# 82magnolia/piccolo

Hardware: AMD Instinct MI355X
Metric: candidate-poses/s (higher is better)
Workload: dtype f32

## Files before the change

__graft_entry__.py:

```python
import os
import sys

REPO = os.path.dirname(os.path.abspath(__file__))
if REPO not in sys.path:
    sys.path.insert(0, REPO)


def build():
    import torch
    from piccolo_amd import build as hip_build
    so = hip_build.build()
    assert os.path.exists(so), so
    assert os.path.exists(hip_build.build_experiments())
    from oracle import oracle as orc
    orc.build()
    from piccolo_amd import _lib
    lib = _lib.load()
    assert lib.pcl_abi_version() == _lib.ABI_VERSION
    import piccolo_amd


def smoke():
    import numpy as np
    import torch
    from oracle import oracle as orc
    from piccolo_amd import _lib, ops, synth
    from piccolo_amd import omniloc as po

    assert torch.cuda.is_available(), "smoke() needs the MI355X"
    _lib.load()
    n, H, W, B = 20_000, 128, 256, 4
    xyz, rgb = synth.box_room(n, 1)
    t_gt, ypr_gt = synth.gt_pose(1)
    dev = torch.device("cuda:0")
    X, C = torch.from_numpy(xyz).to(dev), torch.from_numpy(rgb).to(dev)
    cam = ops.transform_cloud(X, torch.from_numpy(t_gt), torch.from_numpy(ypr_gt))
    img = synth.quantise_like_image_file(ops.make_pano(cam, C, (H, W)))
    trans, rot = synth.start_poses(t_gt, ypr_gt, B, seed=1)

    out = ops.sampling_loss(ops.Cloud(X, C), ops.Pano(img), torch.from_numpy(trans), torch.from_numpy(rot)).cpu().numpy()
    img_host = img.cpu().numpy()
    ref = orc.sampling_loss(xyz, rgb, img_host, trans, rot, dtype=np.float64)
    ref32 = orc.sampling_loss(xyz, rgb, img_host, trans, rot, dtype=np.float32)

    def rel(a, b):
        return np.abs(a - b).max() / np.abs(b).max()

    assert rel(out[:, 0], ref["loss"]) <= 5e-7, (out[:, 0], ref["loss"])
    for key, cols in (("grad_t", slice(2, 5)), ("grad_ypr", slice(5, 8))):
        gap = rel(ref32[key], ref[key])
        err = rel(out[:, cols], ref[key])
        assert err <= 2 * gap + 5e-6, (key, err, gap)

    class Cfg:
        lr, num_iter, patience, factor, out_of_room_quantile, num_input = 0.1, 5, 5, 0.8, 0.05, B

    res = po.omniloc_batch(img, X, C, torch.from_numpy(trans).to(dev), torch.from_numpy(rot).to(dev), Cfg(), {})
    assert res[0].shape == (3, 1) and res[1].shape == (3, 3) and torch.isfinite(res[2])
    print("smoke ok: loss", out[:, 0], "-> refined loss", float(res[2]))


if __name__ == "__main__":
    build()
    if "--smoke" in sys.argv:
        smoke()
```

piccolo_amd/build.py:

```python
import glob
import os
import subprocess
import sys

HERE = os.path.dirname(os.path.abspath(__file__))
CSRC = os.path.join(HERE, "csrc")
OUT_DIR = os.path.join(HERE, "lib")
SO = os.path.join(OUT_DIR, "libpiccolo_hip.so")
ARCH = "gfx950"


def hipcc():
    for c in (os.environ.get("HIPCC"), "/opt/rocm/bin/hipcc", "hipcc"):
        if c and (os.path.isabs(c) and os.path.exists(c) or not os.path.isabs(c)):
            return c
    return "hipcc"


def sources():
    return sorted(glob.glob(os.path.join(CSRC, "*.hip")))


def loss_kernel_source_hash():
    import hashlib
    h = hashlib.sha256()
    for name in ("pcl_loss.hip", "pcl_sample_device.h", "pcl_gd_device.h", "pcl_device.h"):
        with open(os.path.join(CSRC, name), "rb") as f:
            h.update(f.read())
    return h.hexdigest()[:16]


def library_source_hash():
    import hashlib
    h = hashlib.sha256()
    for path in sorted(glob.glob(os.path.join(CSRC, "*.hip")) + glob.glob(os.path.join(CSRC, "*.h"))) + [os.path.join(HERE, "..", "include", "piccolo_hip.h")]:
        with open(path, "rb") as f:
            h.update(f.read())
    return h.hexdigest()[:16]


EXP_SO = os.path.join(OUT_DIR, "libpiccolo_hip_exp.so")
HASH_FILE = "pcl_pack.hip"


def _deps():
    return sources() + glob.glob(os.path.join(CSRC, "*.h")) + [os.path.join(HERE, "..", "include", "piccolo_hip.h")]


def stale(so=None):
    so = so or SO
    if not os.path.exists(so):
        return True
    t = os.path.getmtime(so)
    return any(os.path.getmtime(d) > t for d in _deps())


def build(force=False, verbose=False, extra_flags=(), experiments=False):
    from concurrent.futures import ThreadPoolExecutor
    extra_flags = list(extra_flags) + os.environ.get("PCL_HIPCC_FLAGS", "").split()
    so = EXP_SO if experiments else SO
    if not force and not stale(so):
        return so
    obj_dir = os.path.join(OUT_DIR, "obj_exp" if experiments else "obj")
    os.makedirs(obj_dir, exist_ok=True)
    base = [hipcc(), "--offload-arch=" + ARCH, "-O3", "-std=c++17", "-fPIC", "-fno-gpu-rdc", "-pthread", "-Wall", "-Wno-unused-function"]
    base += (["-DPCL_EXPERIMENTS"] if experiments else []) + extra_flags
    hashes = ['-DPCL_SOURCE_HASH="%s"' % loss_kernel_source_hash(), '-DPCL_LIBRARY_HASH="%s"' % library_source_hash()]
    newest_header = max(os.path.getmtime(d) for d in _deps() if not d.endswith(".hip"))

    def compile_one(src):
        obj = os.path.join(obj_dir, os.path.basename(src)[:-4] + ".o")
        stamped = os.path.basename(src) == HASH_FILE
        if not force and not stamped and not extra_flags and os.path.exists(obj) and os.path.getmtime(obj) > max(os.path.getmtime(src), newest_header):
            return obj
        cmd = base + (hashes if stamped else []) + ["-c", src, "-o", obj]
        if verbose:
            print(" ".join(cmd), flush=True)
        subprocess.check_call(cmd)
        return obj

    with ThreadPoolExecutor(max_workers=min(8, os.cpu_count() or 1)) as pool:
        objs = list(pool.map(compile_one, sources()))
    cmd = [hipcc(), "--offload-arch=" + ARCH, "-shared", "-fPIC", "-fno-gpu-rdc", "-pthread", "-o", so] + objs
    if verbose:
        print(" ".join(cmd), flush=True)
    subprocess.check_call(cmd)
    return so


def build_experiments(force=False, verbose=False):
    return build(force=force, verbose=verbose, experiments=True)


if __name__ == "__main__":
    print(build(force="--force" in sys.argv, verbose=True, experiments="--experiments" in sys.argv))
```

piccolo_amd/csrc/pcl_device.h:

```cpp
#pragma once
#include <hip/hip_runtime.h>
#include <stddef.h>
#include <stdint.h>

#include "../../include/piccolo_hip.h"

#ifdef PCL_EXPERIMENTS
#include <stdlib.h>
static inline int pcl_knob_read(const char* name, int dflt)
{
    const char* v = getenv(name);
    return v && *v ? atoi(v) : dflt;
}
#define PCL_KNOB(NAME, dflt) pcl_knob_read("PCL_" #NAME, (dflt))
#else
#define PCL_KNOB(NAME, dflt) (dflt)
#endif

#define PCL_WAVE 64
#define PCL_BLOCK 256
#define PCL_NACC 8

typedef float pcl_f4 __attribute__((ext_vector_type(4)));
typedef int pcl_i4 __attribute__((ext_vector_type(4)));
typedef int pcl_i2 __attribute__((ext_vector_type(2)));

struct PclPoseRec {
    float R[9];
    float t[3];
    uint32_t pano_lo, pano_hi;
    uint32_t cset;
    float pad;
};
static_assert(sizeof(PclPoseRec) == 64, "pose record is one 64-byte scalar-load line");
static_assert(offsetof(PclPoseRec, R) == 0 && offsetof(PclPoseRec, t) == 36, "pose record: t directly after R[9]");

struct PclGdPose {
    double lr;
    double best;
    float leaf[6];
    float fwd[6];
    float m[6];
    float v[6];
    float last_loss;
    int32_t num_bad;
    int32_t step;
    int32_t pad;
    double beta1_pow, beta2_pow;
    float sc[4];
};
static_assert(sizeof(PclGdPose) == 160, "GD state record");

struct PclDims {
    int H, W;
    int Wp;
    float half_w, half_h;
    float off_x, off_y;
    float k_phi, k_theta;
    float c_scale;
    float k_ix, k_iy;
};

__host__ __device__ inline PclDims pcl_make_dims(int H, int W, int pano_format = PCL_PANO_F32)
{
    PclDims d;
    d.H = H; d.W = W; d.Wp = W + 2;
    d.half_w = 0.5f * (float)W; d.half_h = 0.5f * (float)H;
    d.off_x = 0.5f * (float)(W - 1) + 1.0f; d.off_y = 0.5f * (float)(H - 1) + 1.0f;
    d.k_phi = (float)(-(double)W / (2.0 * 3.14159265358979323846));
    d.k_theta = (float)((double)H / 3.14159265358979323846);
    d.c_scale = 1.0f;
    d.k_ix = (float)(-(double)W / (2.0 * 3.14159265358979323846));
    d.k_iy = (float)(-(double)H / 3.14159265358979323846);
    if (pano_format == PCL_PANO_U8 || pano_format == PCL_PANO_F16) {
        d.k_phi = (float)(-(double)W / (2.0 * 3.14159265358979323846) / 255.0);
        d.k_theta = (float)((double)H / 3.14159265358979323846 / 255.0);
        d.c_scale = (float)(1.0 / 255.0);
    }
    return d;
}

struct PclDepthGrid {
    int Hd, Wd, last;
    float wm1, hm1;
    float tol2;
};
__host__ __device__ inline PclDepthGrid pcl_make_depth_grid(int Hd, int Wd, float tau)
{
    PclDepthGrid g;
    g.Hd = Hd; g.Wd = Wd; g.last = Hd * Wd - 1;
    g.wm1 = (float)(Wd - 1); g.hm1 = (float)(Hd - 1);
    g.tol2 = (1.0f + tau) * (1.0f + tau);
    return g;
}
struct PclDepthLook {
    const uint32_t* zbuf;
    PclDepthGrid grid;
    uint32_t* zclear;
    int64_t zclear_vec4;
};
__device__ inline void pcl_rot_from_ypr(float yaw, float pitch, float roll, float R[9])
{
    double sy, cy, sp, cp, sr, cr;
    sincos((double)yaw, &sy, &cy);
    sincos((double)pitch, &sp, &cp);
    sincos((double)roll, &sr, &cr);
    sy = (double)(float)sy; cy = (double)(float)cy; sp = (double)(float)sp;
    cp = (double)(float)cp; sr = (double)(float)sr; cr = (double)(float)cr;
    R[0] = (float)(cy * cp); R[1] = (float)(cy * sp * sr - sy * cr); R[2] = (float)(cy * sp * cr + sy * sr);
    R[3] = (float)(sy * cp); R[4] = (float)(sy * sp * sr + cy * cr); R[5] = (float)(sy * sp * cr - cy * sr);
    R[6] = (float)(-sp);     R[7] = (float)(cp * sr);                R[8] = (float)(cp * cr);
}

__device__ inline void pcl_write_pose_rec(PclPoseRec* rec, const float p[6])
{
    float R[9];
    pcl_rot_from_ypr(p[3], p[4], p[5], R);
    for (int k = 0; k < 9; k++) rec->R[k] = R[k];
    rec->t[0] = p[0]; rec->t[1] = p[1]; rec->t[2] = p[2];
    rec->pano_lo = 0u; rec->pano_hi = 0u;
    rec->cset = 0u; rec->pad = 0.f;
}

__device__ inline void pcl_write_pose_rec_fast(PclPoseRec* rec, const float p[6], float sc[4])
{
    float sy, cy, sp, cp, sr, cr;
    sincosf(p[3], &sy, &cy);
    sincosf(p[4], &sp, &cp);
    sincosf(p[5], &sr, &cr);
    double dsy = sy, dcy = cy, dsp = sp, dcp = cp, dsr = sr, dcr = cr;
    rec->R[0] = (float)(dcy * dcp); rec->R[1] = (float)(dcy * dsp * dsr - dsy * dcr); rec->R[2] = (float)(dcy * dsp * dcr + dsy * dsr);
    rec->R[3] = (float)(dsy * dcp); rec->R[4] = (float)(dsy * dsp * dsr + dcy * dcr); rec->R[5] = (float)(dsy * dsp * dcr - dcy * dsr);
    rec->R[6] = (float)(-dsp);      rec->R[7] = (float)(dcp * dsr);                   rec->R[8] = (float)(dcp * dcr);
    rec->t[0] = p[0]; rec->t[1] = p[1]; rec->t[2] = p[2];
    sc[0] = sy; sc[1] = cy; sc[2] = sp; sc[3] = cp;
}

__device__ inline void pcl_cloud2idx_point(float px, float py, float pz, float& gx, float& gy)
{
#pragma clang fp contract(off)
    const float pi = 3.14159265358979323846f, two_pi = 6.28318530717958647692f;
    float rho = sqrtf(px * px + py * py);
    float theta = atan2f(rho, pz + 1e-6f);
    float phi = atan2f(py, px + 1e-6f) + pi;
    float cx = 1.0f - phi / two_pi;
    float cy = theta / pi;
    gx = 2.0f * cx - 1.0f;
    gy = 2.0f * cy - 1.0f;
}

__device__ __forceinline__ float pcl_atan_poly(float t)
{
    float s = t * t;
    float p = 2.4566929979e-03f;
    p = fmaf(p, s, -1.4401224869e-02f);
    p = fmaf(p, s, 3.9780993102e-02f);
    p = fmaf(p, s, -7.2348362183e-02f);
    p = fmaf(p, s, 1.0498935044e-01f);
    p = fmaf(p, s, -1.4161225936e-01f);
    p = fmaf(p, s, 1.9985906258e-01f);
    p = fmaf(p, s, -3.3332596993e-01f);
    p = fmaf(p, s, 9.9999988638e-01f);
    return p * t;
}

__device__ __forceinline__ float pcl_atan2(float y, float x)
{
    const float pi = 3.14159265358979323846f, half_pi = 1.57079632679489661923f;
    float ax = fabsf(x), ay = fabsf(y);
    float mx = fmaxf(fmaxf(ax, ay), 1e-37f), mn = fminf(ax, ay);
    float r = pcl_atan_poly(mn * __builtin_amdgcn_rcpf(mx));
    r = ay > ax ? half_pi - r : r;
    r = x < 0.f ? pi - r : r;
    return copysignf(r, y);
}

__device__ __forceinline__ float pcl_atan2_ypos(float y, float x)
{
    const float pi = 3.14159265358979323846f, half_pi = 1.57079632679489661923f;
    float ax = fabsf(x);
    float mx = fmaxf(fmaxf(ax, y), 1e-37f), mn = fminf(ax, y);
    float r = pcl_atan_poly(mn * __builtin_amdgcn_rcpf(mx));
    r = y > ax ? half_pi - r : r;
    return x < 0.f ? pi - r : r;
}

__device__ inline __amdgpu_buffer_rsrc_t pcl_tex_rsrc(const void* pano, int H, int W, int texel_bytes = 16)
{
    return __builtin_amdgcn_make_buffer_rsrc((void*)pano, 0, (int)((size_t)(H + 2) * (size_t)(W + 2) * (size_t)texel_bytes),
                                             0x00020000);
}

__host__ __device__ constexpr int pcl_texel_bytes(int fmt) { return fmt == PCL_PANO_U8 ? 4 : fmt == PCL_PANO_F16 ? 8 : 16; }

__device__ inline pcl_i2 pcl_texel_pair_u8(__amdgpu_buffer_rsrc_t rsrc, int voff, int soff)
{
    return __builtin_amdgcn_raw_buffer_load_b64(rsrc, voff, soff, 0);
}
__device__ __forceinline__ float pcl_ub0(int v) { float f; asm("v_cvt_f32_ubyte0 %0, %1" : "=v"(f) : "v"(v)); return f; }
__device__ __forceinline__ float pcl_ub1(int v) { float f; asm("v_cvt_f32_ubyte1 %0, %1" : "=v"(f) : "v"(v)); return f; }
__device__ __forceinline__ float pcl_ub2(int v) { float f; asm("v_cvt_f32_ubyte2 %0, %1" : "=v"(f) : "v"(v)); return f; }

__device__ inline pcl_f4 pcl_texel(__amdgpu_buffer_rsrc_t rsrc, int voff, int soff)
{
    pcl_i4 v = __builtin_amdgcn_raw_buffer_load_b128(rsrc, voff, soff, 0);
    return __builtin_bit_cast(pcl_f4, v);
}

template <int CTRL>
__device__ __forceinline__ float pcl_dpp(float v)
{
    return __builtin_bit_cast(float, __builtin_amdgcn_update_dpp(0, __builtin_bit_cast(int, v), CTRL, 0xf, 0xf, true));
}
__device__ __forceinline__ float pcl_wave_sum(float v)
{
    v += pcl_dpp<0xB1>(v);
    v += pcl_dpp<0x4E>(v);
    v += pcl_dpp<0x141>(v);
    v += pcl_dpp<0x140>(v);
    float r0 = __builtin_bit_cast(float, __builtin_amdgcn_readlane(__builtin_bit_cast(int, v), 0));
    float r1 = __builtin_bit_cast(float, __builtin_amdgcn_readlane(__builtin_bit_cast(int, v), 16));
    float r2 = __builtin_bit_cast(float, __builtin_amdgcn_readlane(__builtin_bit_cast(int, v), 32));
    float r3 = __builtin_bit_cast(float, __builtin_amdgcn_readlane(__builtin_bit_cast(int, v), 48));
    return (r0 + r1) + (r2 + r3);
}

template <int CTRL>
__device__ __forceinline__ double pcl_dpp_d(double v)
{
    pcl_i2 w = __builtin_bit_cast(pcl_i2, v);
    w.x = __builtin_amdgcn_update_dpp(0, w.x, CTRL, 0xf, 0xf, true);
    w.y = __builtin_amdgcn_update_dpp(0, w.y, CTRL, 0xf, 0xf, true);
    return __builtin_bit_cast(double, w);
}
__device__ __forceinline__ double pcl_readlane_d(double v, int lane)
{
    pcl_i2 w = __builtin_bit_cast(pcl_i2, v);
    w.x = __builtin_amdgcn_readlane(w.x, lane);
    w.y = __builtin_amdgcn_readlane(w.y, lane);
    return __builtin_bit_cast(double, w);
}
__device__ __forceinline__ double pcl_wave_sum_d(double v)
{
    v += pcl_dpp_d<0xB1>(v);
    v += pcl_dpp_d<0x4E>(v);
    v += pcl_dpp_d<0x141>(v);
    v += pcl_dpp_d<0x140>(v);
    return (pcl_readlane_d(v, 0) + pcl_readlane_d(v, 16)) + (pcl_readlane_d(v, 32) + pcl_readlane_d(v, 48));
}

#define PCL_LAUNCH_CHECK()                         \
    do {                                           \
        hipError_t e_ = hipGetLastError();         \
        if (e_ != hipSuccess) return (int)e_;      \
    } while (0)
```

piccolo_amd/csrc/pcl_loss.hip:

```cpp
#include <stdlib.h>

#include "pcl_gd_device.h"
#include "pcl_sample_device.h"

struct PclLossArgs {
    const float* cloud;
    int64_t n, stride;
    const void* pano;
    PclDims dims;
    const PclPoseRec* poses;
    int B;
    const uint8_t* visible;
    const uint32_t* zbuf;
    PclDepthGrid dgrid;
    pcl_i4* zclear;
    int zclear_per_block;
    int64_t zclear_total;
    float* partials;
    int nchunks;
    int ngroups;
    int flip;
    int seg_len;
    int xcd_groups;
    int steps_base, steps_rem;
    int color_sets;
};

#define PCL_STEP (2 * PCL_BLOCK)

#ifdef PCL_BLOCK_TRACE
__device__ unsigned long long* pcl_trace_buf = nullptr;
extern "C" int pcl_debug_set_block_trace(unsigned long long* buf)
{
    return (int)hipMemcpyToSymbol(HIP_SYMBOL(pcl_trace_buf), &buf, sizeof(buf));
}
#define PCL_TRACE_NOW() __builtin_amdgcn_s_memrealtime()
__global__ void pcl_debug_stamp_kernel(unsigned long long* slot) { *slot = PCL_TRACE_NOW(); }
extern "C" int pcl_debug_stamp(unsigned long long* slot, void* stream)
{
    hipLaunchKernelGGL(pcl_debug_stamp_kernel, dim3(1), dim3(1), 0, (hipStream_t)stream, slot);
    return (int)hipGetLastError();
}
#endif

template <int G, bool FUSED>
__device__ __forceinline__ unsigned pcl_room_select(const PclLossArgs& a_in, const PclFuseArgs& f_in, const PclRoomTable* __restrict__ tb, PclLossArgs& a,
                                                    PclFuseArgs& f)
{
    int r = -1;
#pragma unroll
    for (int q = 0; q < PCL_GD_MAX_ROOMS; q++) r += (int)blockIdx.x >= pcl_rfl(tb->block0[q]) ? 1 : 0;
    const PclRoomRec* __restrict__ rm = tb->rec + r;
    const int group0 = pcl_rfl(rm->group0), pose0 = group0 * G;
    const long long poff = (long long)pcl_rfl64((unsigned long long)rm->partials);
    a = a_in;
    a.cloud = (const float*)pcl_rfl64(rm->cloud);
    a.n = pcl_rfl(rm->n); a.stride = pcl_rfl(rm->stride);
    a.nchunks = pcl_rfl(rm->nchunks); a.seg_len = pcl_rfl(rm->seg_len);
    a.steps_base = pcl_rfl(rm->steps_base); a.steps_rem = pcl_rfl(rm->steps_rem);
    a.poses = a_in.poses + pose0;
    a.partials = a_in.partials + poff;
    a.xcd_groups = 0;
    f = f_in;
    if constexpr (FUSED) {
        f.partials_in = f_in.partials_in + poff;
        f.st_in = f_in.st_in + pose0; f.recs_in = f_in.recs_in + pose0;
        f.st_out = f_in.st_out + pose0; f.recs_out = f_in.recs_out + pose0;
        f.box = (const float*)pcl_rfl64(rm->box);
        f.loss_out = f_in.loss_out ? f_in.loss_out + pose0 : nullptr;
    }
    return blockIdx.x - (unsigned)pcl_rfl(rm->block0);
}

template <int G, bool GRAD, int VIS, int FMT, bool FUSED, bool CS = false, bool RM = false>
__device__ __forceinline__ void pcl_loss_body(const PclLossArgs& a_in, const PclFuseArgs& f_in, const PclRoomTable* rooms = nullptr)
{
    PclLossArgs a_rm;
    PclFuseArgs f_rm;
    unsigned bid = blockIdx.x;
    if constexpr (RM) bid = pcl_room_select<G, FUSED>(a_in, f_in, rooms, a_rm, f_rm);
    const PclLossArgs& a = RM ? a_rm : a_in;
    const PclFuseArgs& f = RM ? f_rm : f_in;
    int group, chunk;
    if (a.xcd_groups) {
        const int gpx = a.ngroups >> 3, j = (int)(bid >> 3), cj = j / gpx;
        group = (int)(bid & 7) * gpx + (j - cj * gpx);
        chunk = a.flip ? a.nchunks - 1 - cj : cj;
    } else {
        const int lq = (int)(bid >> 3) / a.ngroups;
        group = (int)(bid >> 3) - lq * a.ngroups;
        const int lc = a.flip ? (a.nchunks >> 3) - 1 - lq : lq;
        const int run = lc / a.seg_len;
        chunk = (run * 8 + (int)(bid & 7)) * a.seg_len + (lc - run * a.seg_len);
    }
    const int pose0 = group * G;

    PclPose6 P6[G];
    unsigned PANO[G][2];
    __amdgpu_buffer_rsrc_t tex = pcl_tex_rsrc(a.pano, a.dims.H, a.dims.W, pcl_texel_bytes(FMT));
    __amdgpu_buffer_rsrc_t cld = __builtin_amdgcn_make_buffer_rsrc((void*)a.cloud, 0, CS ? (int)(a.stride * (3 + 3 * a.color_sets) * 4) : (int)(a.stride * 6 * 4),
                                                                   0x00020000);
    const int plane = (int)a.stride * 4;
    int cplane = 3 * plane;
    if constexpr (CS) cplane = (int)(3u + 3u * (unsigned)__builtin_amdgcn_readfirstlane((int)(a.poses + pose0)->cset)) * plane;
    __amdgpu_buffer_rsrc_t zb = __amdgpu_buffer_rsrc_t();
    if constexpr (VIS == 2) zb = __builtin_amdgcn_make_buffer_rsrc((void*)a.zbuf, 0, (int)((unsigned)a.B * (unsigned)(a.dgrid.last + 1) * 4u), 0x00020000);

    f2 acc[G][PCL_NACC];
    int count[G];
#pragma unroll
    for (int g = 0; g < G; g++) {
        count[g] = 0;
#pragma unroll
        for (int k = 0; k < PCL_NACC; k++) acc[g][k] = F2(0.f);
    }

    int first = chunk * a.steps_base + min(chunk, a.steps_rem);
    int nsteps = a.steps_base + (chunk < a.steps_rem ? 1 : 0);
    const int begin = first * PCL_STEP;
    int end = begin + nsteps * PCL_STEP;
    if (end > (int)a.n) end = (int)a.n;
    const int last = (int)a.n - 1;

    auto load_step = [&](int base, float (&dst)[2][6]) {
        int j0 = min(base + (int)threadIdx.x, last), j1 = min(base + PCL_BLOCK + (int)threadIdx.x, last);
#pragma unroll
        for (int k = 0; k < 6; k++) {
            const int soff = (CS && k >= 3) ? cplane + (k - 3) * plane : k * plane;
            dst[0][k] = __builtin_bit_cast(float, __builtin_amdgcn_raw_buffer_load_b32(cld, j0 * 4, soff, 0));
            dst[1][k] = __builtin_bit_cast(float, __builtin_amdgcn_raw_buffer_load_b32(cld, j1 * 4, soff, 0));
        }
    };
    auto eval_step = [&](int base, const float (&src)[2][6]) {
        const int i0 = base + threadIdx.x, i1 = i0 + PCL_BLOCK;
        const bool valid0 = i0 < end, valid1 = i1 < end;
        const unsigned long long vmask0 = __builtin_amdgcn_ballot_w64(valid0), vmask1 = __builtin_amdgcn_ballot_w64(valid1);
        f2 x = {src[0][0], src[1][0]}, y = {src[0][1], src[1][1]}, z = {src[0][2], src[1][2]};
        f2 ncr = {src[0][3], src[1][3]}, ncg = {src[0][4], src[1][4]}, ncb = {src[0][5], src[1][5]};
#ifndef PCL_NO_ROTATE_PAIR
        f2 rot_p[G][3];
#ifdef PCL_TIMING_ONLY_NO_ROTATION
        if constexpr (G == 2) {
            const f2 oa = F2((a.poses + pose0)->t[0]), ob = F2((a.poses + pose0 + 1)->t[0]);
            rot_p[0][0] = x - oa; rot_p[0][1] = y; rot_p[0][2] = z;
            rot_p[1][0] = x - ob; rot_p[1][1] = y; rot_p[1][2] = z;
        } else
#endif
        if constexpr (G == 2) {
            if constexpr (FUSED) pcl_rotate2x2(x, y, z, P6[0], P6[1], rot_p[0][0], rot_p[0][1], rot_p[0][2], rot_p[1][0], rot_p[1][1], rot_p[1][2]);
            else pcl_rotate2x2(x, y, z, pcl_pose6(a.poses + pose0), pcl_pose6(a.poses + pose0 + 1), rot_p[0][0], rot_p[0][1], rot_p[0][2],
                               rot_p[1][0], rot_p[1][1], rot_p[1][2]);
        }
#endif
#pragma unroll
        for (int g = 0; g < G; g++) {
            const PclPoseRec* __restrict__ pr = a.poses + (pose0 + g);
            bool ok0 = valid0, ok1 = valid1;
            unsigned long long m0 = vmask0, m1 = vmask1;
            if constexpr (VIS == 1) {
                const uint8_t* vis = a.visible + (int64_t)(pose0 + g) * a.n;
                ok0 = ok0 && vis[min(i0, last)] != 0;
                ok1 = ok1 && vis[min(i1, last)] != 0;
                m0 = __builtin_amdgcn_ballot_w64(ok0); m1 = __builtin_amdgcn_ballot_w64(ok1);
            }
            __amdgpu_buffer_rsrc_t tg = tex;
            unsigned pano_lo = pr->pano_lo, pano_hi = pr->pano_hi;
            if constexpr (FUSED) {
                pano_lo = PANO[g][0]; pano_hi = PANO[g][1];
            }
            if (pano_lo | pano_hi) {
                const void* pp = (const void*)(((unsigned long long)pano_hi << 32) | (unsigned long long)pano_lo);
                tg = pcl_tex_rsrc(pp, a.dims.H, a.dims.W, pcl_texel_bytes(FMT));
            }
            PclProj<FMT> pj;
            const int zoff = VIS == 2 ? (int)((unsigned)(pose0 + g) * (unsigned)(a.dgrid.last + 1) * 4u) : 0;
#ifndef PCL_NO_ROTATE_PAIR
            if constexpr (G == 2) {
                pj.px = rot_p[g][0]; pj.py = rot_p[g][1]; pj.pz = rot_p[g][2];
                pcl_project2_rotated<FMT, VIS == 2>(tg, a.dims, pj, zb, zoff, &a.dgrid);
            } else
#endif
            if constexpr (FUSED) pcl_project2<FMT, VIS == 2>(x, y, z, P6[g], tg, a.dims, pj, zb, zoff, &a.dgrid);
            else pcl_project2<FMT, VIS == 2>(x, y, z, pcl_pose6(pr), tg, a.dims, pj, zb, zoff, &a.dgrid);
            if constexpr (VIS == 2) {
                f2 d2 = pcl_fma2(pj.pz, pj.pz, pj.rho2);
                const bool v0 = d2.x <= __uint_as_float(pj.zq0), v1 = d2.y <= __uint_as_float(pj.zq1);
                ok0 = ok0 & v0; ok1 = ok1 & v1;
                m0 = __builtin_amdgcn_ballot_w64(ok0); m1 = __builtin_amdgcn_ballot_w64(ok1);
            }
            pcl_sample2<GRAD, FMT>(pj, ncr, ncg, ncb, ok0, ok1, m0, m1, tg, a.dims, acc[g], count[g]);
        }
    };
    float bufA[2][6], bufB[2][6];
    load_step(begin, bufA);
    if constexpr (FUSED) {
        static_assert(PCL_BLOCK == PCL_GD_THREADS, "the fused prologue reduces with the epilogue kernel's thread layout");
        __shared__ double gd_rows[(PCL_GD_THREADS / 16) * 2 * G][4];
        __shared__ double gd_sums[G][PCL_NACC];
        __shared__ float pose_sh[G][12];
        pcl_gd_finish_group<G, true>(f.partials_in, a.nchunks, group, (int)threadIdx.x, f.st_in, f.recs_in, f.st_out, f.recs_out, chunk == 0,
                                     f.box, f.factor, f.patience, f.mode, f.loss_out, gd_rows, gd_sums, pose_sh);
        __syncthreads();
#pragma unroll
        for (int g = 0; g < G; g++) {
            float v[12];
#pragma unroll
            for (int k = 0; k < 12; k++) v[k] = __builtin_bit_cast(float, __builtin_amdgcn_readfirstlane(__builtin_bit_cast(int, pose_sh[g][k])));
            P6[g] = PclPose6{(f2){v[0], v[1]}, (f2){v[2], v[3]}, (f2){v[4], v[5]}, (f2){v[6], v[7]}, (f2){v[8], v[9]}, (f2){v[10], v[11]}};
            const PclPoseRec* pr = a.poses + (pose0 + g);
            PANO[g][0] = (unsigned)__builtin_amdgcn_readfirstlane((int)pr->pano_lo);
            PANO[g][1] = (unsigned)__builtin_amdgcn_readfirstlane((int)pr->pano_hi);
        }
    }

    for (int base = begin; base < end; base += 2 * PCL_STEP) {
        load_step(base + PCL_STEP, bufB);
        eval_step(base, bufA);
        if (base + PCL_STEP < end) {
            load_step(base + 2 * PCL_STEP, bufA);
            eval_step(base + PCL_STEP, bufB);
        }
    }

    __shared__ float red[PCL_BLOCK / PCL_WAVE][G * PCL_NACC];
    const int lane = threadIdx.x & 63, wave = threadIdx.x >> 6;
#pragma unroll
    for (int g = 0; g < G; g++)
#pragma unroll
        for (int k = 0; k < PCL_NACC; k++) {
            if (k == 1) {
                if (lane == 0) red[wave][g * PCL_NACC + 1] = (float)count[g];
                continue;
            }
            if (!GRAD && k >= 2) continue;
            float s = pcl_wave_sum(acc[g][k].x + acc[g][k].y);
            if (lane == 0) red[wave][g * PCL_NACC + k] = s;
        }
    __syncthreads();
    if (threadIdx.x < G * PCL_NACC) {
        int g = threadIdx.x / PCL_NACC, k = threadIdx.x - g * PCL_NACC;
        float s = 0.f;
        if (GRAD || k < 2) s = red[0][threadIdx.x] + red[1][threadIdx.x] + red[2][threadIdx.x] + red[3][threadIdx.x];
        a.partials[pcl_partials_row(a.nchunks, G, group, chunk, g) + k] = s;
    }
    if constexpr (VIS == 2) {
        if (a.zclear) {
            const pcl_i4 inf4 = {0x7f800000, 0x7f800000, 0x7f800000, 0x7f800000};
            const int64_t z0 = (int64_t)blockIdx.x * a.zclear_per_block;
            for (int i = threadIdx.x; i < a.zclear_per_block; i += PCL_BLOCK)
                if (z0 + i < a.zclear_total) a.zclear[z0 + i] = inf4;
        }
    }
#ifdef PCL_BLOCK_TRACE
    if (pcl_trace_buf && threadIdx.x == 0) {
        unsigned hw, xcc;
        asm volatile("s_getreg_b32 %0, hwreg(HW_REG_HW_ID)" : "=s"(hw));
        asm volatile("s_getreg_b32 %0, hwreg(HW_REG_XCC_ID)" : "=s"(xcc));
        unsigned long long* t = pcl_trace_buf + (size_t)blockIdx.x * 4;
        t[0] = 0; t[1] = 0; t[2] = PCL_TRACE_NOW(); t[3] = ((unsigned long long)xcc << 32) | hw;
    }
#endif
}

template <int G, bool GRAD, int VIS, int FMT>
__global__ void __launch_bounds__(PCL_BLOCK) pcl_loss_kernel(PclLossArgs a)
{
    pcl_loss_body<G, GRAD, VIS, FMT, false>(a, PclFuseArgs{});
}

template <int G, int FMT>
__global__ void __launch_bounds__(PCL_BLOCK) pcl_loss_fused_kernel(PclLossArgs a, PclFuseArgs f)
{
    pcl_loss_body<G, true, 0, FMT, true>(a, f);
}

template <int G, int FMT>
__global__ void __launch_bounds__(PCL_BLOCK) pcl_loss_sets_kernel(PclLossArgs a)
{
    pcl_loss_body<G, true, 0, FMT, false, true>(a, PclFuseArgs{});
}

template <int G, int FMT>
__global__ void __launch_bounds__(PCL_BLOCK) pcl_loss_fused_sets_kernel(PclLossArgs a, PclFuseArgs f)
{
    pcl_loss_body<G, true, 0, FMT, true, true>(a, f);
}

template <int G, int FMT>
__global__ void __launch_bounds__(PCL_BLOCK) pcl_loss_rooms_kernel(PclLossArgs a, const PclRoomTable* rooms)
{
    pcl_loss_body<G, true, 0, FMT, false, false, true>(a, PclFuseArgs{}, rooms);
}

template <int G, int FMT>
__global__ void __launch_bounds__(PCL_BLOCK) pcl_loss_fused_rooms_kernel(PclLossArgs a, PclFuseArgs f, const PclRoomTable* rooms)
{
    pcl_loss_body<G, true, 0, FMT, true, false, true>(a, f, rooms);
}



struct PclPlan {
    int G, ngroups, nchunks;
    int seg_len;
    int steps_base, steps_rem;
};

static int pcl_xcd_seg_len(int nchunks, int64_t nblocks)
{
    static const int runs_env = PCL_KNOB(XCD_RUNS, 0);
    int cpx = nchunks / 8, runs = runs_env < 1 || runs_env > cpx ? cpx : runs_env;
    if (runs_env < 1 && nblocks <= 1024) runs = 1;
    while (cpx % runs) runs--;
    return cpx / runs;
}

static PclPlan pcl_plan(int64_t n, int B)
{
    static const int g_env = PCL_KNOB(G, 0), blocks_env = PCL_KNOB(BLOCKS, 4096);
    PclPlan p;
    p.G = (B % 2 == 0) ? 2 : 1;
    if (g_env > 0 && B % g_env == 0) p.G = g_env;
    p.ngroups = B / p.G;
    int64_t want = blocks_env / p.ngroups;
    if (want < 64) want = 64;
    if (n > 2000000 && want < n / 8192) want = n / 8192;
    int64_t steps = (n + PCL_STEP - 1) / PCL_STEP;
    if (steps < 3 * want) {
        int64_t alt = steps / 3;
        if (alt < 1024 / p.ngroups) alt = 1024 / p.ngroups;
        if (alt < 32) alt = 32;
        if (alt < want) want = alt;
    }
    if (want > steps) want = steps;
    want = ((want + 7) / 8) * 8;
    p.nchunks = (int)want;
    p.steps_base = (int)(steps / want);
    p.steps_rem = (int)(steps % want);
    p.seg_len = pcl_xcd_seg_len(p.nchunks, (int64_t)p.nchunks * p.ngroups);
    return p;
}

static PclPlan pcl_plan_sets(int64_t n, int B, int sets)
{
    if (sets <= 1) return pcl_plan(n, B);
    PclPlan p = pcl_plan(n, B / sets);
    p.ngroups = B / p.G;
    p.seg_len = pcl_xcd_seg_len(p.nchunks, (int64_t)p.nchunks * p.ngroups);
    return p;
}

void pcl_plan_room(int64_t n, int per_room, int* G, int* ngroups, int* nchunks, int* seg_len, int* steps_base, int* steps_rem)
{
    const PclPlan p = pcl_plan(n, per_room);
    *G = p.G; *ngroups = p.ngroups; *nchunks = p.nchunks; *seg_len = p.seg_len; *steps_base = p.steps_base; *steps_rem = p.steps_rem;
}

size_t pcl_partials_bytes(int64_t n, int B, int sets)
{
    PclPlan p = pcl_plan_sets(n, B, sets);
    return (size_t)p.nchunks * (size_t)B * PCL_NACC * sizeof(float);
}

int pcl_plan_nchunks(int64_t n, int B, int sets) { return pcl_plan_sets(n, B, sets).nchunks; }
int pcl_plan_nblocks(int64_t n, int B, int sets) { PclPlan p = pcl_plan_sets(n, B, sets); return p.nchunks * p.ngroups; }
int pcl_plan_G(int64_t n, int B, int sets) { return pcl_plan_sets(n, B, sets).G; }

void pcl_plan_for_groups(int64_t n, int ngroups, int* nchunks, int* seg_len, int* steps_base, int* steps_rem)
{
    PclPlan p = pcl_plan(n, 2 * ngroups);
    static const int chunks_env = PCL_KNOB(TRIM_CHUNKS, 0);
    int auto_chunks = 0;
    const int64_t per_chunk = n <= 2000000 ? 8192 : 16384;
    if (chunks_env < 8 && n > 64 * per_chunk) auto_chunks = (int)((n + per_chunk - 1) / per_chunk);
    if (chunks_env >= 8 || auto_chunks) {
        int64_t steps = (n + PCL_STEP - 1) / PCL_STEP, want = (((chunks_env >= 8 ? chunks_env : auto_chunks) + 7) / 8) * 8;
        if (want > steps) want = ((steps + 7) / 8) * 8;
        p.nchunks = (int)want; p.steps_base = (int)(steps / want); p.steps_rem = (int)(steps % want);
        static const int runs_env = PCL_KNOB(TRIM_RUNS, 0);
        int cpx = p.nchunks / 8, runs = runs_env < 1 || runs_env > cpx ? cpx : runs_env;
        while (cpx % runs) runs--;
        p.seg_len = cpx / runs;
    }
    *nchunks = p.nchunks; *seg_len = p.seg_len; *steps_base = p.steps_base; *steps_rem = p.steps_rem;
}

template <int G, int FMT>
static void pcl_launch_g(const PclLossArgs& a, int nblk, bool grad, int vis, hipStream_t s)
{
    if (grad) {
        if (vis == 2) hipLaunchKernelGGL((pcl_loss_kernel<G, true, 2, FMT>), dim3(nblk), dim3(PCL_BLOCK), 0, s, a);
        else if (vis) hipLaunchKernelGGL((pcl_loss_kernel<G, true, 1, FMT>), dim3(nblk), dim3(PCL_BLOCK), 0, s, a);
        else hipLaunchKernelGGL((pcl_loss_kernel<G, true, 0, FMT>), dim3(nblk), dim3(PCL_BLOCK), 0, s, a);
    } else {
        if (vis == 2) hipLaunchKernelGGL((pcl_loss_kernel<G, false, 2, FMT>), dim3(nblk), dim3(PCL_BLOCK), 0, s, a);
        else if (vis) hipLaunchKernelGGL((pcl_loss_kernel<G, false, 1, FMT>), dim3(nblk), dim3(PCL_BLOCK), 0, s, a);
        else hipLaunchKernelGGL((pcl_loss_kernel<G, false, 0, FMT>), dim3(nblk), dim3(PCL_BLOCK), 0, s, a);
    }
}

template <int FMT>
static void pcl_launch_f(const PclLossArgs& a, int G, int nblk, bool grad, int vis, hipStream_t s)
{
    if (G == 4) pcl_launch_g<4, FMT>(a, nblk, grad, vis, s);
    else if (G == 2) pcl_launch_g<2, FMT>(a, nblk, grad, vis, s);
    else pcl_launch_g<1, FMT>(a, nblk, grad, vis, s);
}

template <int FMT>
static void pcl_launch_fused(const PclLossArgs& a, const PclFuseArgs& f, int G, int nblk, hipStream_t s)
{
    if (G == 4) hipLaunchKernelGGL((pcl_loss_fused_kernel<4, FMT>), dim3(nblk), dim3(PCL_BLOCK), 0, s, a, f);
    else if (G == 2) hipLaunchKernelGGL((pcl_loss_fused_kernel<2, FMT>), dim3(nblk), dim3(PCL_BLOCK), 0, s, a, f);
    else hipLaunchKernelGGL((pcl_loss_fused_kernel<1, FMT>), dim3(nblk), dim3(PCL_BLOCK), 0, s, a, f);
}

template <int FMT>
static void pcl_launch_sets(const PclLossArgs& a, const PclFuseArgs* f, int G, int nblk, hipStream_t s)
{
    if (f) {
        if (G == 4) hipLaunchKernelGGL((pcl_loss_fused_sets_kernel<4, FMT>), dim3(nblk), dim3(PCL_BLOCK), 0, s, a, *f);
        else if (G == 2) hipLaunchKernelGGL((pcl_loss_fused_sets_kernel<2, FMT>), dim3(nblk), dim3(PCL_BLOCK), 0, s, a, *f);
        else hipLaunchKernelGGL((pcl_loss_fused_sets_kernel<1, FMT>), dim3(nblk), dim3(PCL_BLOCK), 0, s, a, *f);
    } else {
        if (G == 4) hipLaunchKernelGGL((pcl_loss_sets_kernel<4, FMT>), dim3(nblk), dim3(PCL_BLOCK), 0, s, a);
        else if (G == 2) hipLaunchKernelGGL((pcl_loss_sets_kernel<2, FMT>), dim3(nblk), dim3(PCL_BLOCK), 0, s, a);
        else hipLaunchKernelGGL((pcl_loss_sets_kernel<1, FMT>), dim3(nblk), dim3(PCL_BLOCK), 0, s, a);
    }
}

int pcl_launch_loss_rooms(const PclRoomTable* rooms, const void* pano, int pano_format, int H, int W, const PclPoseRec* poses, int B, int G,
                          int ngroups, int nblk, float* partials, hipStream_t s, int flip, const PclFuseArgs* fuse)
{
    if (pano_format != PCL_PANO_F32 && pano_format != PCL_PANO_U8 && pano_format != PCL_PANO_F16) return PCL_EINVAL;
    if ((int64_t)(H + 2) * (W + 2) * pcl_texel_bytes(pano_format) >= ((int64_t)1 << 31)) return PCL_EINVAL;
    PclLossArgs a = PclLossArgs{};
    a.pano = pano; a.dims = pcl_make_dims(H, W, pano_format);
    a.poses = poses; a.B = B; a.partials = partials;
    a.ngroups = ngroups; a.flip = flip & 1; a.xcd_groups = 0; a.color_sets = 1;
    const dim3 grid(nblk), blk(PCL_BLOCK);
    if (fuse) {
        if (pano_format == PCL_PANO_U8) {
            if (G == 2) hipLaunchKernelGGL((pcl_loss_fused_rooms_kernel<2, PCL_PANO_U8>), grid, blk, 0, s, a, *fuse, rooms);
            else hipLaunchKernelGGL((pcl_loss_fused_rooms_kernel<1, PCL_PANO_U8>), grid, blk, 0, s, a, *fuse, rooms);
        } else if (pano_format == PCL_PANO_F16) {
            if (G == 2) hipLaunchKernelGGL((pcl_loss_fused_rooms_kernel<2, PCL_PANO_F16>), grid, blk, 0, s, a, *fuse, rooms);
            else hipLaunchKernelGGL((pcl_loss_fused_rooms_kernel<1, PCL_PANO_F16>), grid, blk, 0, s, a, *fuse, rooms);
        } else {
            if (G == 2) hipLaunchKernelGGL((pcl_loss_fused_rooms_kernel<2, PCL_PANO_F32>), grid, blk, 0, s, a, *fuse, rooms);
            else hipLaunchKernelGGL((pcl_loss_fused_rooms_kernel<1, PCL_PANO_F32>), grid, blk, 0, s, a, *fuse, rooms);
        }
    } else {
        if (pano_format == PCL_PANO_U8) {
            if (G == 2) hipLaunchKernelGGL((pcl_loss_rooms_kernel<2, PCL_PANO_U8>), grid, blk, 0, s, a, rooms);
            else hipLaunchKernelGGL((pcl_loss_rooms_kernel<1, PCL_PANO_U8>), grid, blk, 0, s, a, rooms);
        } else if (pano_format == PCL_PANO_F16) {
            if (G == 2) hipLaunchKernelGGL((pcl_loss_rooms_kernel<2, PCL_PANO_F16>), grid, blk, 0, s, a, rooms);
            else hipLaunchKernelGGL((pcl_loss_rooms_kernel<1, PCL_PANO_F16>), grid, blk, 0, s, a, rooms);
        } else {
            if (G == 2) hipLaunchKernelGGL((pcl_loss_rooms_kernel<2, PCL_PANO_F32>), grid, blk, 0, s, a, rooms);
            else hipLaunchKernelGGL((pcl_loss_rooms_kernel<1, PCL_PANO_F32>), grid, blk, 0, s, a, rooms);
        }
    }
    PCL_LAUNCH_CHECK();
    return 0;
}

int pcl_launch_loss(const float* cloud, int64_t n, const void* pano, int pano_format, int H, int W, const PclPoseRec* poses,
                    int B, bool grad, const uint8_t* visible, float* partials, hipStream_t s, int flip, const PclFuseArgs* fuse,
                    const PclDepthLook* depth, int color_sets)
{
    if (pano_format != PCL_PANO_F32 && pano_format != PCL_PANO_U8 && pano_format != PCL_PANO_F16) return PCL_EINVAL;
    if (n > PCL_MAX_POINTS || (int64_t)(H + 2) * (W + 2) * pcl_texel_bytes(pano_format) >= ((int64_t)1 << 31)) return PCL_EINVAL;
    const bool sets = color_sets > 1;
    if (sets && (B % color_sets || !grad || visible || depth || pcl_cloud_sets_bytes(n, color_sets) == 0)) return PCL_EINVAL;
    PclPlan p = pcl_plan_sets(n, B, color_sets);
    PclLossArgs a;
    a.cloud = cloud; a.n = n; a.stride = pcl_cloud_stride(n);
    a.pano = pano; a.dims = pcl_make_dims(H, W, pano_format);
    a.poses = poses; a.B = B; a.visible = visible; a.partials = partials;
    a.zbuf = nullptr; a.dgrid = PclDepthGrid{};
    a.zclear = nullptr; a.zclear_per_block = 0; a.zclear_total = 0;
    if (depth) {
        if (visible || !depth->zbuf || depth->grid.Hd <= 0 || depth->grid.Wd <= 0) return PCL_EINVAL;
        if ((int64_t)B * depth->grid.Hd * depth->grid.Wd * 4 >= ((int64_t)1 << 32)) return PCL_EINVAL;
        a.zbuf = depth->zbuf; a.dgrid = depth->grid;
        if (depth->zclear) {
            const int64_t nblk64 = (int64_t)p.nchunks * p.ngroups;
            a.zclear = (pcl_i4*)depth->zclear;
            a.zclear_total = depth->zclear_vec4;
            a.zclear_per_block = (int)((depth->zclear_vec4 + nblk64 - 1) / nblk64);
        }
    }
    a.nchunks = p.nchunks; a.ngroups = p.ngroups; a.seg_len = p.seg_len; a.flip = flip & 1; a.steps_base = p.steps_base; a.steps_rem = p.steps_rem;
    a.color_sets = sets ? color_sets : 1;
    static const int xg_env = PCL_KNOB(XCD_GROUPS, -1);
    a.xcd_groups = ((flip & 2) != 0 || xg_env == 1) && xg_env != 0 && p.ngroups % 8 == 0 ? 1 : 0;
    int nblk = p.nchunks * p.ngroups;
    const int vis = depth ? 2 : visible != nullptr ? 1 : 0;
    if (sets) {
        if (pano_format == PCL_PANO_U8) pcl_launch_sets<PCL_PANO_U8>(a, fuse, p.G, nblk, s);
        else if (pano_format == PCL_PANO_F16) pcl_launch_sets<PCL_PANO_F16>(a, fuse, p.G, nblk, s);
        else pcl_launch_sets<PCL_PANO_F32>(a, fuse, p.G, nblk, s);
        PCL_LAUNCH_CHECK();
        return 0;
    }
    if (fuse) {
        if (!grad || vis) return PCL_EINVAL;
        if (pano_format == PCL_PANO_U8) pcl_launch_fused<PCL_PANO_U8>(a, *fuse, p.G, nblk, s);
        else if (pano_format == PCL_PANO_F16) pcl_launch_fused<PCL_PANO_F16>(a, *fuse, p.G, nblk, s);
        else pcl_launch_fused<PCL_PANO_F32>(a, *fuse, p.G, nblk, s);
        PCL_LAUNCH_CHECK();
        return 0;
    }
    if (pano_format == PCL_PANO_U8) pcl_launch_f<PCL_PANO_U8>(a, p.G, nblk, grad, vis, s);
    else if (pano_format == PCL_PANO_F16) pcl_launch_f<PCL_PANO_F16>(a, p.G, nblk, grad, vis, s);
    else pcl_launch_f<PCL_PANO_F32>(a, p.G, nblk, grad, vis, s);
    PCL_LAUNCH_CHECK();
    return 0;
}
```

piccolo_amd/csrc/pcl_pack.hip:

```cpp
#include "pcl_device.h"

#include <rocprim/device/device_radix_sort.hpp>

extern "C" int pcl_abi_version(void) { return PCL_ABI_VERSION; }

#ifndef PCL_SOURCE_HASH
#define PCL_SOURCE_HASH "unstamped"
#endif
extern "C" const char* pcl_source_hash(void) { return PCL_SOURCE_HASH; }
#ifndef PCL_LIBRARY_HASH
#define PCL_LIBRARY_HASH "unstamped"
#endif
extern "C" const char* pcl_library_hash(void) { return PCL_LIBRARY_HASH; }

extern "C" const char* pcl_error_string(int code)
{
    if (code == 0) return "success";
    if (code == PCL_EINVAL) return "piccolo_hip: invalid argument";
    if (code == PCL_EWORKSPACE) return "piccolo_hip: workspace too small";
    if (code > 0) return hipGetErrorString((hipError_t)code);
    return "piccolo_hip: unknown error";
}

extern "C" int64_t pcl_cloud_stride(int64_t n) { return n <= 0 ? 0 : ((n + 255) / 256) * 256; }
extern "C" size_t pcl_cloud_bytes(int64_t n) { return (size_t)pcl_cloud_stride(n) * 6 * sizeof(float); }
extern "C" size_t pcl_pano_bytes(int H, int W, int pano_format)
{
    if (H <= 0 || W <= 0) return 0;
    if (pano_format == PCL_PANO_U8P) return (size_t)((H + 3) >> 1) * (size_t)(W + 2) * 8;
    if (pano_format == PCL_PANO_U8V) return (size_t)(H + 2) * (size_t)(W + 2) * 8;
    if (pano_format != PCL_PANO_F32 && pano_format != PCL_PANO_U8 && pano_format != PCL_PANO_F16) return 0;
    return (size_t)(H + 2) * (size_t)(W + 2) * (size_t)pcl_texel_bytes(pano_format);
}

__global__ void __launch_bounds__(PCL_BLOCK) pcl_cloud_pack_kernel(const float* __restrict__ xyz, const float* __restrict__ rgb,
                                                                   const int64_t* __restrict__ order, int64_t n,
                                                                   int64_t stride, float* __restrict__ cloud)
{
    int64_t i = (int64_t)blockIdx.x * PCL_BLOCK + threadIdx.x;
    if (i >= stride) return;
    float v[6] = {0.f, 0.f, 0.f, 0.f, 0.f, 0.f};
    if (i < n) {
        int64_t j = order ? order[i] : i;
        v[0] = xyz[3 * j]; v[1] = xyz[3 * j + 1]; v[2] = xyz[3 * j + 2];
        v[3] = -rgb[3 * j]; v[4] = -rgb[3 * j + 1]; v[5] = -rgb[3 * j + 2];
    }
#pragma unroll
    for (int k = 0; k < 6; k++) cloud[k * stride + i] = v[k];
}

extern "C" int pcl_cloud_pack(const float* xyz, const float* rgb, const int64_t* order, int64_t n, float* cloud, void* stream)
{
    if (!xyz || !rgb || !cloud || n <= 0) return PCL_EINVAL;
    int64_t stride = pcl_cloud_stride(n);
    hipLaunchKernelGGL(pcl_cloud_pack_kernel, dim3((unsigned)(stride / PCL_BLOCK)), dim3(PCL_BLOCK), 0, (hipStream_t)stream,
                       xyz, rgb, order, n, stride, cloud);
    PCL_LAUNCH_CHECK();
    return 0;
}

extern "C" size_t pcl_cloud_sets_bytes(int64_t n, int nsets)
{
    if (n <= 0 || n > PCL_MAX_POINTS || nsets <= 0) return 0;
    if (nsets == 1) return pcl_cloud_bytes(n);
    const int64_t bytes = (int64_t)pcl_cloud_stride(n) * 4 * (3 + 3 * (int64_t)nsets);
    return bytes < ((int64_t)1 << 31) ? (size_t)bytes : 0;
}

#define PCL_PACK_SETS 16
struct PclRgbList { const float* p[PCL_PACK_SETS]; };

__global__ void __launch_bounds__(PCL_BLOCK) pcl_cloud_pack_sets_kernel(const float* __restrict__ xyz, PclRgbList rgb, int k0, int m,
                                                                        const int64_t* __restrict__ order, int64_t n, int64_t stride,
                                                                        float* __restrict__ cloud)
{
    int64_t i = (int64_t)blockIdx.x * PCL_BLOCK + threadIdx.x;
    if (i >= stride) return;
    const int64_t j = i < n ? (order ? order[i] : i) : 0;
    if (k0 == 0)
        for (int c = 0; c < 3; c++) cloud[c * stride + i] = i < n ? xyz[3 * j + c] : 0.f;
    for (int k = 0; k < m; k++)
        for (int c = 0; c < 3; c++) cloud[(3 + 3 * (int64_t)(k0 + k) + c) * stride + i] = i < n ? -rgb.p[k][3 * j + c] : 0.f;
}

extern "C" int pcl_cloud_pack_sets(const float* xyz, const float* const* rgb_host, int nsets, const int64_t* order, int64_t n, float* cloud,
                                   void* stream)
{
    if (!xyz || !rgb_host || !cloud || n <= 0 || nsets <= 0) return PCL_EINVAL;
    if (pcl_cloud_sets_bytes(n, nsets) == 0) return PCL_EINVAL;
    for (int k = 0; k < nsets; k++)
        if (!rgb_host[k]) return PCL_EINVAL;
    if (nsets == 1) return pcl_cloud_pack(xyz, rgb_host[0], order, n, cloud, stream);
    const int64_t stride = pcl_cloud_stride(n);
    for (int k0 = 0; k0 < nsets; k0 += PCL_PACK_SETS) {
        const int m = nsets - k0 < PCL_PACK_SETS ? nsets - k0 : PCL_PACK_SETS;
        PclRgbList l;
        for (int k = 0; k < PCL_PACK_SETS; k++) l.p[k] = k < m ? rgb_host[k0 + k] : nullptr;
        hipLaunchKernelGGL(pcl_cloud_pack_sets_kernel, dim3((unsigned)(stride / PCL_BLOCK)), dim3(PCL_BLOCK), 0, (hipStream_t)stream, xyz, l, k0, m,
                           order, n, stride, cloud);
        PCL_LAUNCH_CHECK();
    }
    return 0;
}

__device__ inline uint64_t pcl_spread21(uint32_t v)
{
    uint64_t x = v & 0x1fffffu;
    x = (x | x << 32) & 0x1f00000000ffffull;
    x = (x | x << 16) & 0x1f0000ff0000ffull;
    x = (x | x << 8) & 0x100f00f00f00f00full;
    x = (x | x << 4) & 0x10c30c30c30c30c3ull;
    x = (x | x << 2) & 0x1249249249249249ull;
    return x;
}

__global__ void __launch_bounds__(PCL_BLOCK) pcl_morton_kernel(const float* __restrict__ xyz, int64_t n, float lx, float ly,
                                                               float lz, float sx, float sy, float sz,
                                                               int64_t* __restrict__ keys)
{
    int64_t i = (int64_t)blockIdx.x * PCL_BLOCK + threadIdx.x;
    if (i >= n) return;
    const float top = 2097151.f;
    float fx = __builtin_amdgcn_fmed3f((xyz[3 * i] - lx) * sx, 0.f, top);
    float fy = __builtin_amdgcn_fmed3f((xyz[3 * i + 1] - ly) * sy, 0.f, top);
    float fz = __builtin_amdgcn_fmed3f((xyz[3 * i + 2] - lz) * sz, 0.f, top);
    uint64_t k = pcl_spread21((uint32_t)fx) | (pcl_spread21((uint32_t)fy) << 1) | (pcl_spread21((uint32_t)fz) << 2);
    keys[i] = (int64_t)k;
}

extern "C" int pcl_morton_keys(const float* xyz, int64_t n, const float* lo, const float* hi, int64_t* keys, void* stream)
{
    if (!xyz || !lo || !hi || !keys || n <= 0) return PCL_EINVAL;
    float s[3];
    for (int k = 0; k < 3; k++) s[k] = hi[k] > lo[k] ? 2097151.f / (hi[k] - lo[k]) : 0.f;
    hipLaunchKernelGGL(pcl_morton_kernel, dim3((unsigned)((n + PCL_BLOCK - 1) / PCL_BLOCK)), dim3(PCL_BLOCK), 0,
                       (hipStream_t)stream, xyz, n, lo[0], lo[1], lo[2], s[0], s[1], s[2], keys);
    PCL_LAUNCH_CHECK();
    return 0;
}

__device__ __forceinline__ unsigned int pcl_ordered_key(float v)
{
    unsigned int b = __float_as_uint(v);
    return (b & 0x80000000u) ? ~b : (b | 0x80000000u);
}
__device__ __forceinline__ float pcl_ordered_value(unsigned int k)
{
    return __uint_as_float((k & 0x80000000u) ? (k & 0x7fffffffu) : ~k);
}

__global__ void __launch_bounds__(PCL_BLOCK) pcl_bbox_kernel(const float* __restrict__ xyz, int64_t n, unsigned int* __restrict__ box)
{
    unsigned int lo[3] = {~0u, ~0u, ~0u}, hi[3] = {0u, 0u, 0u};
    for (int64_t i = (int64_t)blockIdx.x * PCL_BLOCK + threadIdx.x; i < n; i += (int64_t)gridDim.x * PCL_BLOCK) {
#pragma unroll
        for (int c = 0; c < 3; c++) {
            unsigned int k = pcl_ordered_key(xyz[3 * i + c]);
            lo[c] = min(lo[c], k); hi[c] = max(hi[c], k);
        }
    }
#pragma unroll
    for (int c = 0; c < 3; c++) {
#pragma unroll
        for (int o = 32; o > 0; o >>= 1) {
            lo[c] = min(lo[c], (unsigned int)__shfl_xor((int)lo[c], o, 64));
            hi[c] = max(hi[c], (unsigned int)__shfl_xor((int)hi[c], o, 64));
        }
        if ((threadIdx.x & 63) == 0) { atomicMin(&box[c], lo[c]); atomicMax(&box[3 + c], hi[c]); }
    }
}

__global__ void __launch_bounds__(PCL_BLOCK) pcl_morton_box_kernel(const float* __restrict__ xyz, int64_t n, const unsigned int* __restrict__ box,
                                                                   unsigned long long* __restrict__ keys, int64_t* __restrict__ iota)
{
    int64_t i = (int64_t)blockIdx.x * PCL_BLOCK + threadIdx.x;
    if (i >= n) return;
    const float top = 2097151.f;
    unsigned long long k = 0ull;
#pragma unroll
    for (int c = 0; c < 3; c++) {
        float lo = pcl_ordered_value(box[c]), hi = pcl_ordered_value(box[3 + c]);
        float sc = hi > lo ? top / (hi - lo) : 0.f;
        float f = __builtin_amdgcn_fmed3f((xyz[3 * i + c] - lo) * sc, 0.f, top);
        k |= pcl_spread21((uint32_t)f) << c;
    }
    keys[i] = k;
    iota[i] = i;
}

static size_t order_align(size_t v) { return (v + 255) & ~(size_t)255; }
static size_t order_sort_temp_bytes(int64_t n)
{
    size_t bytes = 0;
    (void)rocprim::radix_sort_pairs<rocprim::default_config, const unsigned long long*, unsigned long long*, const int64_t*, int64_t*>(
        nullptr, bytes, nullptr, nullptr, nullptr, nullptr, (size_t)n, 0, 63, nullptr, false);
    return bytes;
}

extern "C" size_t pcl_cloud_order_workspace_bytes(int64_t n)
{
    if (n <= 0) return 0;
    return order_align(64) + 3 * order_align((size_t)n * 8) + order_align(order_sort_temp_bytes(n));
}

extern "C" int pcl_cloud_order(const float* xyz, int64_t n, int64_t* order, void* workspace, size_t workspace_bytes, void* stream)
{
    if (!xyz || !order || !workspace || n <= 0 || n > PCL_MAX_POINTS) return PCL_EINVAL;
    if (workspace_bytes < pcl_cloud_order_workspace_bytes(n)) return PCL_EWORKSPACE;
    hipStream_t s = (hipStream_t)stream;
    char* ws = (char*)workspace;
    unsigned int* box = (unsigned int*)ws; ws += order_align(64);
    unsigned long long* keys = (unsigned long long*)ws; ws += order_align((size_t)n * 8);
    unsigned long long* keys_sorted = (unsigned long long*)ws; ws += order_align((size_t)n * 8);
    int64_t* iota = (int64_t*)ws; ws += order_align((size_t)n * 8);
    hipError_t e = hipMemsetAsync(box, 0xff, 12, s);
    if (e == hipSuccess) e = hipMemsetAsync(box + 3, 0, 12, s);
    if (e != hipSuccess) return (int)e;
    int64_t blocks = (n + PCL_BLOCK - 1) / PCL_BLOCK;
    hipLaunchKernelGGL(pcl_bbox_kernel, dim3((unsigned)(blocks < 1024 ? blocks : 1024)), dim3(PCL_BLOCK), 0, s, xyz, n, box);
    hipLaunchKernelGGL(pcl_morton_box_kernel, dim3((unsigned)blocks), dim3(PCL_BLOCK), 0, s, xyz, n, box, keys, iota);
    PCL_LAUNCH_CHECK();
    size_t temp_bytes = order_sort_temp_bytes(n);
    e = rocprim::radix_sort_pairs(ws, temp_bytes, (const unsigned long long*)keys, keys_sorted, (const int64_t*)iota, order, (size_t)n, 0, 63,
                                  s, false);
    return e == hipSuccess ? 0 : (int)e;
}

__global__ void __launch_bounds__(PCL_BLOCK) pcl_pano_pack_kernel(const float* __restrict__ img, int H, int W,
                                                                  pcl_f4* __restrict__ pano)
{
    int Wp = W + 2, Hp = H + 2;
    int64_t i = (int64_t)blockIdx.x * PCL_BLOCK + threadIdx.x;
    if (i >= (int64_t)Wp * Hp) return;
    int yp = (int)(i / Wp), xp = (int)(i - (int64_t)yp * Wp);
    pcl_f4 v = {0.f, 0.f, 0.f, 0.f};
    if (yp >= 1 && yp <= H && xp >= 1 && xp <= W) {
        const float* s = img + ((int64_t)(yp - 1) * W + (xp - 1)) * 3;
        v.x = s[0]; v.y = s[1]; v.z = s[2];
    }
    pano[i] = v;
}

extern "C" int pcl_pano_pack(const float* img_hwc, int H, int W, float* pano, void* stream)
{
    if (!img_hwc || !pano || H <= 0 || W <= 0) return PCL_EINVAL;
    int64_t total = (int64_t)(H + 2) * (W + 2);
    hipLaunchKernelGGL(pcl_pano_pack_kernel, dim3((unsigned)((total + PCL_BLOCK - 1) / PCL_BLOCK)), dim3(PCL_BLOCK), 0,
                       (hipStream_t)stream, img_hwc, H, W, (pcl_f4*)pano);
    PCL_LAUNCH_CHECK();
    return 0;
}

__global__ void __launch_bounds__(PCL_BLOCK) pcl_pano_pack_u8_kernel(const float* __restrict__ img, int H, int W,
                                                                     uint32_t* __restrict__ pano, int* __restrict__ not_exact)
{
    int Wp = W + 2, Hp = H + 2;
    int64_t i = (int64_t)blockIdx.x * PCL_BLOCK + threadIdx.x;
    if (i >= (int64_t)Wp * Hp) return;
    int yp = (int)(i / Wp), xp = (int)(i - (int64_t)yp * Wp);
    uint32_t v = 0u;
    if (yp >= 1 && yp <= H && xp >= 1 && xp <= W) {
        const float* s = img + ((int64_t)(yp - 1) * W + (xp - 1)) * 3;
        bool bad = false;
#pragma unroll
        for (int c = 0; c < 3; c++) {
            float f = s[c], k = rintf(f * 255.f);
            bad = bad || !(k >= 0.f && k <= 255.f) || __fdiv_rn(k, 255.f) != f;
            v |= ((uint32_t)k & 255u) << (8 * c);
        }
        if (bad) *not_exact = 1;
    }
    pano[i] = v;
}

__global__ void __launch_bounds__(PCL_BLOCK) pcl_pano_pack_u8p_kernel(const float* __restrict__ img, int H, int W,
                                                                      uint32_t* __restrict__ pano, int* __restrict__ not_exact)
{
    const int Wp = W + 2, pairs = (H + 3) >> 1;
    int64_t i = (int64_t)blockIdx.x * PCL_BLOCK + threadIdx.x;
    if (i >= (int64_t)Wp * pairs * 2) return;
    const int yp = (int)(i / Wp), xp = (int)(i - (int64_t)yp * Wp);
    uint32_t v = 0u;
    if (yp >= 1 && yp <= H && xp >= 1 && xp <= W) {
        const float* s = img + ((int64_t)(yp - 1) * W + (xp - 1)) * 3;
        bool bad = false;
#pragma unroll
        for (int c = 0; c < 3; c++) {
            float f = s[c], k = rintf(f * 255.f);
            bad = bad || !(k >= 0.f && k <= 255.f) || __fdiv_rn(k, 255.f) != f;
            v |= ((uint32_t)k & 255u) << (8 * c);
        }
        if (bad) *not_exact = 1;
    }
    pano[((int64_t)(yp >> 1) * Wp + xp) * 2 + (yp & 1)] = v;
}

__global__ void __launch_bounds__(PCL_BLOCK) pcl_pano_pack_u8v_kernel(const float* __restrict__ img, int H, int W,
                                                                      pcl_i2* __restrict__ pano, int* __restrict__ not_exact)
{
    const int Wp = W + 2, Hp = H + 2;
    int64_t i = (int64_t)blockIdx.x * PCL_BLOCK + threadIdx.x;
    if (i >= (int64_t)Wp * Hp) return;
    const int yp = (int)(i / Wp), xp = (int)(i - (int64_t)yp * Wp);
    uint32_t v[2] = {0u, 0u};
    bool bad = false;
#pragma unroll
    for (int d = 0; d < 2; d++) {
        const int y = yp + d;
        if (y >= 1 && y <= H && xp >= 1 && xp <= W) {
            const float* s = img + ((int64_t)(y - 1) * W + (xp - 1)) * 3;
#pragma unroll
            for (int c = 0; c < 3; c++) {
                float f = s[c], k = rintf(f * 255.f);
                bad = bad || !(k >= 0.f && k <= 255.f) || __fdiv_rn(k, 255.f) != f;
                v[d] |= ((uint32_t)k & 255u) << (8 * c);
            }
        }
    }
    if (bad) *not_exact = 1;
    pano[i] = (pcl_i2){(int)v[0], (int)v[1]};
}

extern "C" int pcl_pano_pack_u8v(const float* img_hwc, int H, int W, uint32_t* pano, int* not_exact, void* stream)
{
    if (!img_hwc || !pano || !not_exact || H <= 0 || W <= 0) return PCL_EINVAL;
    int64_t total = (int64_t)(H + 2) * (W + 2);
    hipLaunchKernelGGL(pcl_pano_pack_u8v_kernel, dim3((unsigned)((total + PCL_BLOCK - 1) / PCL_BLOCK)), dim3(PCL_BLOCK), 0,
                       (hipStream_t)stream, img_hwc, H, W, (pcl_i2*)pano, not_exact);
    PCL_LAUNCH_CHECK();
    return 0;
}

__global__ void __launch_bounds__(PCL_BLOCK) pcl_pano_pack_f16_kernel(const float* __restrict__ img, int H, int W,
                                                                      pcl_i2* __restrict__ pano, int* __restrict__ not_exact)
{
    typedef _Float16 h2 __attribute__((ext_vector_type(2)));
    int Wp = W + 2, Hp = H + 2;
    int64_t i = (int64_t)blockIdx.x * PCL_BLOCK + threadIdx.x;
    if (i >= (int64_t)Wp * Hp) return;
    int yp = (int)(i / Wp), xp = (int)(i - (int64_t)yp * Wp);
    float lv[3] = {0.f, 0.f, 0.f};
    if (yp >= 1 && yp <= H && xp >= 1 && xp <= W) {
        const float* s = img + ((int64_t)(yp - 1) * W + (xp - 1)) * 3;
        bool bad = false;
#pragma unroll
        for (int c = 0; c < 3; c++) {
            float f = s[c], k = rintf(f * 255.f);
            bad = bad || !(k >= 0.f && k <= 255.f) || __fdiv_rn(k, 255.f) != f;
            lv[c] = k;
        }
        if (bad) *not_exact = 1;
    }
    h2 rg = {(_Float16)lv[0], (_Float16)lv[1]}, b0 = {(_Float16)lv[2], (_Float16)0.f};
    pano[i] = (pcl_i2){__builtin_bit_cast(int, rg), __builtin_bit_cast(int, b0)};
}

extern "C" int pcl_pano_pack_f16(const float* img_hwc, int H, int W, void* pano, int* not_exact, void* stream)
{
    if (!img_hwc || !pano || !not_exact || H <= 0 || W <= 0) return PCL_EINVAL;
    int64_t total = (int64_t)(H + 2) * (W + 2);
    hipLaunchKernelGGL(pcl_pano_pack_f16_kernel, dim3((unsigned)((total + PCL_BLOCK - 1) / PCL_BLOCK)), dim3(PCL_BLOCK), 0,
                       (hipStream_t)stream, img_hwc, H, W, (pcl_i2*)pano, not_exact);
    PCL_LAUNCH_CHECK();
    return 0;
}

extern "C" int pcl_pano_pack_u8p(const float* img_hwc, int H, int W, uint32_t* pano, int* not_exact, void* stream)
{
    if (!img_hwc || !pano || !not_exact || H <= 0 || W <= 0) return PCL_EINVAL;
    int64_t total = (int64_t)((H + 3) >> 1) * 2 * (W + 2);
    hipLaunchKernelGGL(pcl_pano_pack_u8p_kernel, dim3((unsigned)((total + PCL_BLOCK - 1) / PCL_BLOCK)), dim3(PCL_BLOCK), 0,
                       (hipStream_t)stream, img_hwc, H, W, pano, not_exact);
    PCL_LAUNCH_CHECK();
    return 0;
}

extern "C" int pcl_pano_pack_u8(const float* img_hwc, int H, int W, uint32_t* pano, int* not_exact, void* stream)
{
    if (!img_hwc || !pano || !not_exact || H <= 0 || W <= 0) return PCL_EINVAL;
    int64_t total = (int64_t)(H + 2) * (W + 2);
    hipLaunchKernelGGL(pcl_pano_pack_u8_kernel, dim3((unsigned)((total + PCL_BLOCK - 1) / PCL_BLOCK)), dim3(PCL_BLOCK), 0,
                       (hipStream_t)stream, img_hwc, H, W, pano, not_exact);
    PCL_LAUNCH_CHECK();
    return 0;
}
```

piccolo_amd/csrc/pcl_sample_device.h:

```cpp
#pragma once
#include "pcl_device.h"

typedef float f2 __attribute__((ext_vector_type(2)));
#define F2(s) ((f2){(s), (s)})

__device__ __forceinline__ f2 pcl_fma2(f2 a, f2 b, f2 c) { return __builtin_elementwise_fma(a, b, c); }

__device__ __forceinline__ f2 pcl_atan_poly2(f2 t)
{
    f2 s = t * t;
    f2 p = F2(2.4566929979e-03f);
    p = pcl_fma2(p, s, F2(-1.4401224869e-02f));
    p = pcl_fma2(p, s, F2(3.9780993102e-02f));
    p = pcl_fma2(p, s, F2(-7.2348362183e-02f));
    p = pcl_fma2(p, s, F2(1.0498935044e-01f));
    p = pcl_fma2(p, s, F2(-1.4161225936e-01f));
    p = pcl_fma2(p, s, F2(1.9985906258e-01f));
    p = pcl_fma2(p, s, F2(-3.3332596993e-01f));
    p = pcl_fma2(p, s, F2(9.9999988638e-01f));
    return p * t;
}

__device__ __forceinline__ float pcl_min_abs(float a, float b)
{
    float r;
    asm("v_min_f32_e64 %0, |%1|, |%2|" : "=v"(r) : "v"(a), "v"(b));
    return r;
}
__device__ __forceinline__ f2 pcl_atan_ratio2(float u0, float v0, float u1, float v1)
{
    f2 mn = {pcl_min_abs(u0, v0), pcl_min_abs(u1, v1)};
    f2 rc = {__builtin_amdgcn_rcpf(fmaxf(fmaxf(fabsf(u0), fabsf(v0)), 1e-37f)), __builtin_amdgcn_rcpf(fmaxf(fmaxf(fabsf(u1), fabsf(v1)), 1e-37f))};
    return pcl_atan_poly2(mn * rc);
}

__device__ __forceinline__ f2 pcl_atan2_2(f2 y, f2 x)
{
    const float half_pi = 1.57079632679489661923f;
    float ax0 = fabsf(x.x), ax1 = fabsf(x.y), ay0 = fabsf(y.x), ay1 = fabsf(y.y);
    f2 r = pcl_atan_ratio2(x.x, y.x, x.y, y.y);
    f2 alt = F2(half_pi) - r;
    r = (f2){ay0 > ax0 ? alt.x : r.x, ay1 > ax1 ? alt.y : r.y};
    f2 w = F2(half_pi) - r;
    w = (f2){copysignf(w.x, x.x), copysignf(w.y, x.y)};
    r = F2(half_pi) - w;
    return (f2){copysignf(r.x, y.x), copysignf(r.y, y.y)};
}

__device__ __forceinline__ f2 pcl_elevation2(f2 z, f2 rho)
{
    const float half_pi = 1.57079632679489661923f;
    float az0 = fabsf(z.x), az1 = fabsf(z.y);
    f2 r = pcl_atan_ratio2(rho.x, z.x, rho.y, z.y);
    f2 alt = F2(half_pi) - r;
    r = (f2){az0 > rho.x ? alt.x : r.x, az1 > rho.y ? alt.y : r.y};
    return (f2){copysignf(r.x, z.x), copysignf(r.y, z.y)};
}

template <int FMT> struct PclTaps;
template <> struct PclTaps<PCL_PANO_U8> { pcl_i2 top, bot; };
template <> struct PclTaps<PCL_PANO_F32> { int voff, row; };
template <> struct PclTaps<PCL_PANO_F16> { pcl_i4 top, bot; };

__device__ __forceinline__ void pcl_issue_taps(__amdgpu_buffer_rsrc_t tex, int x0, int y0, int Wp, PclTaps<PCL_PANO_U8>& o)
{
    int voff = (int)(__umul24((unsigned)y0, (unsigned)Wp) + (unsigned)x0) * 4;
    o.top = pcl_texel_pair_u8(tex, voff, 0);
    o.bot = pcl_texel_pair_u8(tex, voff, Wp * 4);
}
__device__ __forceinline__ void pcl_issue_taps(__amdgpu_buffer_rsrc_t tex, int x0, int y0, int Wp, PclTaps<PCL_PANO_F16>& o)
{
    int voff = (int)(__umul24((unsigned)y0, (unsigned)Wp) + (unsigned)x0) * 8;
    o.top = __builtin_amdgcn_raw_buffer_load_b128(tex, voff, 0, 0);
    o.bot = __builtin_amdgcn_raw_buffer_load_b128(tex, voff, Wp * 8, 0);
}
__device__ __forceinline__ void pcl_issue_taps(__amdgpu_buffer_rsrc_t tex, int x0, int y0, int Wp, PclTaps<PCL_PANO_F32>& o)
{
    o.voff = (int)(__umul24((unsigned)y0, (unsigned)Wp) + (unsigned)x0) * 16;
    o.row = Wp * 16;
}
__device__ __forceinline__ void pcl_unpack_taps(__amdgpu_buffer_rsrc_t, const PclTaps<PCL_PANO_U8>& r, float t[12])
{
    t[0] = pcl_ub0(r.top.x); t[1] = pcl_ub1(r.top.x); t[2] = pcl_ub2(r.top.x);
    t[3] = pcl_ub0(r.top.y); t[4] = pcl_ub1(r.top.y); t[5] = pcl_ub2(r.top.y);
    t[6] = pcl_ub0(r.bot.x); t[7] = pcl_ub1(r.bot.x); t[8] = pcl_ub2(r.bot.x);
    t[9] = pcl_ub0(r.bot.y); t[10] = pcl_ub1(r.bot.y); t[11] = pcl_ub2(r.bot.y);
}
__device__ __forceinline__ void pcl_unpack_taps(__amdgpu_buffer_rsrc_t tex, const PclTaps<PCL_PANO_F32>& r, float t[12])
{
    pcl_f4 t00 = pcl_texel(tex, r.voff, 0), t01 = pcl_texel(tex, r.voff + 16, 0);
    pcl_f4 t10 = pcl_texel(tex, r.voff, r.row), t11 = pcl_texel(tex, r.voff + 16, r.row);
    t[0] = t00.x; t[1] = t00.y; t[2] = t00.z; t[3] = t01.x; t[4] = t01.y; t[5] = t01.z;
    t[6] = t10.x; t[7] = t10.y; t[8] = t10.z; t[9] = t11.x; t[10] = t11.y; t[11] = t11.z;
}

typedef _Float16 pcl_h2 __attribute__((ext_vector_type(2)));
__device__ __forceinline__ float pcl_mix_lo(float a, pcl_h2 b, pcl_h2 c)
{
    float r;
    asm("v_fma_mix_f32 %0, %1, %2, %3 op_sel:[0,0,0] op_sel_hi:[0,1,1]" : "=v"(r) : "v"(a), "v"(b), "v"(c));
    return r;
}
__device__ __forceinline__ float pcl_mix_hi(float a, pcl_h2 b, pcl_h2 c)
{
    float r;
    asm("v_fma_mix_f32 %0, %1, %2, %3 op_sel:[0,1,1] op_sel_hi:[0,1,1]" : "=v"(r) : "v"(a), "v"(b), "v"(c));
    return r;
}
struct PclBilerp1 { float top[3], bot[3], dh[3]; };
template <bool GRAD>
__device__ __forceinline__ void pcl_bilerp_f16(const PclTaps<PCL_PANO_F16>& r, float fx, float fy, PclBilerp1& o)
{
    typedef _Float16 pcl_h8 __attribute__((ext_vector_type(8)));
    pcl_h8 tv = __builtin_bit_cast(pcl_h8, r.top), bv = __builtin_bit_cast(pcl_h8, r.bot);
    pcl_h2 t00a = __builtin_shufflevector(tv, tv, 0, 1), t00b = __builtin_shufflevector(tv, tv, 2, 3);
    pcl_h2 t01a = __builtin_shufflevector(tv, tv, 4, 5), t01b = __builtin_shufflevector(tv, tv, 6, 7);
    pcl_h2 t10a = __builtin_shufflevector(bv, bv, 0, 1), t10b = __builtin_shufflevector(bv, bv, 2, 3);
    pcl_h2 t11a = __builtin_shufflevector(bv, bv, 4, 5), t11b = __builtin_shufflevector(bv, bv, 6, 7);
    pcl_h2 dta = t01a - t00a, dtb = t01b - t00b, dba = t11a - t10a, dbb = t11b - t10b;
    o.top[0] = pcl_mix_lo(fx, dta, t00a); o.bot[0] = pcl_mix_lo(fx, dba, t10a);
    o.top[1] = pcl_mix_hi(fx, dta, t00a); o.bot[1] = pcl_mix_hi(fx, dba, t10a);
    o.top[2] = pcl_mix_lo(fx, dtb, t00b); o.bot[2] = pcl_mix_lo(fx, dbb, t10b);
    if (GRAD) {
        pcl_h2 dda = dba - dta, ddb = dbb - dtb;
        o.dh[0] = pcl_mix_lo(fy, dda, dta);
        o.dh[1] = pcl_mix_hi(fy, dda, dta);
        o.dh[2] = pcl_mix_lo(fy, ddb, dtb);
    }
}

template <int FMT>
struct PclProj {
    f2 px, py, pz;
    f2 rho2, rinv;
    f2 rs2;
    f2 fx, fy;
    bool in_phi0, in_phi1, in_th0, in_th1;
    PclTaps<FMT> ta, tb;
    unsigned zq0, zq1;
};

__device__ __forceinline__ void pcl_depth_cells2(f2 phi, f2 hel, const PclDepthGrid& g, int& row0, int& col0, int& row1, int& col1)
{
    const float inv_2pi = 0.15915494309189532f;
    f2 colf = pcl_fma2(-phi, F2(inv_2pi), F2(0.5f)) * F2(g.wm1);
    f2 rowf = pcl_fma2(-(hel * F2(4.0f)), F2(inv_2pi), F2(0.5f)) * F2(g.hm1);
    row0 = (int)rowf.x; col0 = (int)colf.x; row1 = (int)rowf.y; col1 = (int)colf.y;
}

struct PclPose6 { f2 p0, p1, p2, p3, p4, p5; };
__device__ __forceinline__ PclPose6 pcl_pose6(const PclPoseRec* __restrict__ pose)
{
    const f2* __restrict__ P = reinterpret_cast<const f2*>(pose->R);
    return PclPose6{P[0], P[1], P[2], P[3], P[4], P[5]};
}
__device__ __forceinline__ void pcl_rotate2(f2 x, f2 y, f2 z, const PclPose6& P, f2& opx, f2& opy, f2& opz)
{
    const f2 p0 = P.p0, p1 = P.p1, p2 = P.p2, p3 = P.p3, p4 = P.p4, p5 = P.p5;
    f2 qx, qy, qz, px, py, pz;
    asm("v_pk_add_f32 %3, %6, %13 op_sel:[0,1] op_sel_hi:[1,1] neg_lo:[0,1] neg_hi:[0,1]\n\t"
        "v_pk_add_f32 %4, %7, %14 op_sel_hi:[1,0] neg_lo:[0,1] neg_hi:[0,1]\n\t"
        "v_pk_add_f32 %5, %8, %14 op_sel:[0,1] op_sel_hi:[1,1] neg_lo:[0,1] neg_hi:[0,1]\n\t"
        "v_pk_mul_f32 %0, %3, %9 op_sel_hi:[1,0]\n\t"
        "v_pk_mul_f32 %1, %3, %10 op_sel:[0,1] op_sel_hi:[1,1]\n\t"
        "v_pk_mul_f32 %2, %3, %12 op_sel_hi:[1,0]\n\t"
        "v_pk_fma_f32 %0, %9, %4, %0 op_sel:[1,0,0] op_sel_hi:[1,1,1]\n\t"
        "v_pk_fma_f32 %1, %11, %4, %1 op_sel_hi:[0,1,1]\n\t"
        "v_pk_fma_f32 %2, %12, %4, %2 op_sel:[1,0,0] op_sel_hi:[1,1,1]\n\t"
        "v_pk_fma_f32 %0, %10, %5, %0 op_sel_hi:[0,1,1]\n\t"
        "v_pk_fma_f32 %1, %11, %5, %1 op_sel:[1,0,0] op_sel_hi:[1,1,1]\n\t"
        "v_pk_fma_f32 %2, %13, %5, %2 op_sel_hi:[0,1,1]\n\t"
        "s_nop 0"
        : "=&v"(px), "=&v"(py), "=&v"(pz), "=&v"(qx), "=&v"(qy), "=&v"(qz)
        : "v"(x), "v"(y), "v"(z), "s"(p0), "s"(p1), "s"(p2), "s"(p3), "s"(p4), "s"(p5));
    opx = px; opy = py; opz = pz;
}
#ifndef PCL_NO_ROTATE_PAIR
__device__ __forceinline__ void pcl_rotate2x2(f2 x, f2 y, f2 z, const PclPose6& A, const PclPose6& B, f2& apx, f2& apy, f2& apz, f2& bpx,
                                              f2& bpy, f2& bpz)
{
    f2 aqx, aqy, aqz, bqx, bqy, bqz, ax, ay, az, bx, by, bz;
    asm("v_pk_add_f32 %6, %12, %19 op_sel:[0,1] op_sel_hi:[1,1] neg_lo:[0,1] neg_hi:[0,1]\n\t"
        "v_pk_add_f32 %9, %12, %25 op_sel:[0,1] op_sel_hi:[1,1] neg_lo:[0,1] neg_hi:[0,1]\n\t"
        "v_pk_add_f32 %7, %13, %20 op_sel_hi:[1,0] neg_lo:[0,1] neg_hi:[0,1]\n\t"
        "v_pk_add_f32 %10, %13, %26 op_sel_hi:[1,0] neg_lo:[0,1] neg_hi:[0,1]\n\t"
        "v_pk_add_f32 %8, %14, %20 op_sel:[0,1] op_sel_hi:[1,1] neg_lo:[0,1] neg_hi:[0,1]\n\t"
        "v_pk_add_f32 %11, %14, %26 op_sel:[0,1] op_sel_hi:[1,1] neg_lo:[0,1] neg_hi:[0,1]\n\t"
        "v_pk_mul_f32 %0, %6, %15 op_sel_hi:[1,0]\n\t"
        "v_pk_mul_f32 %3, %9, %21 op_sel_hi:[1,0]\n\t"
        "v_pk_mul_f32 %1, %6, %16 op_sel:[0,1] op_sel_hi:[1,1]\n\t"
        "v_pk_mul_f32 %4, %9, %22 op_sel:[0,1] op_sel_hi:[1,1]\n\t"
        "v_pk_mul_f32 %2, %6, %18 op_sel_hi:[1,0]\n\t"
        "v_pk_mul_f32 %5, %9, %24 op_sel_hi:[1,0]\n\t"
        "v_pk_fma_f32 %0, %15, %7, %0 op_sel:[1,0,0] op_sel_hi:[1,1,1]\n\t"
        "v_pk_fma_f32 %3, %21, %10, %3 op_sel:[1,0,0] op_sel_hi:[1,1,1]\n\t"
        "v_pk_fma_f32 %1, %17, %7, %1 op_sel_hi:[0,1,1]\n\t"
        "v_pk_fma_f32 %4, %23, %10, %4 op_sel_hi:[0,1,1]\n\t"
        "v_pk_fma_f32 %2, %18, %7, %2 op_sel:[1,0,0] op_sel_hi:[1,1,1]\n\t"
        "v_pk_fma_f32 %5, %24, %10, %5 op_sel:[1,0,0] op_sel_hi:[1,1,1]\n\t"
        "v_pk_fma_f32 %0, %16, %8, %0 op_sel_hi:[0,1,1]\n\t"
        "v_pk_fma_f32 %3, %22, %11, %3 op_sel_hi:[0,1,1]\n\t"
        "v_pk_fma_f32 %1, %17, %8, %1 op_sel:[1,0,0] op_sel_hi:[1,1,1]\n\t"
        "v_pk_fma_f32 %4, %23, %11, %4 op_sel:[1,0,0] op_sel_hi:[1,1,1]\n\t"
        "v_pk_fma_f32 %2, %19, %8, %2 op_sel_hi:[0,1,1]\n\t"
        "v_pk_fma_f32 %5, %25, %11, %5 op_sel_hi:[0,1,1]\n\t"
        "s_nop 0"
        : "=&v"(ax), "=&v"(ay), "=&v"(az), "=&v"(bx), "=&v"(by), "=&v"(bz), "=&v"(aqx), "=&v"(aqy), "=&v"(aqz), "=&v"(bqx), "=&v"(bqy), "=&v"(bqz)
        : "v"(x), "v"(y), "v"(z), "s"(A.p0), "s"(A.p1), "s"(A.p2), "s"(A.p3), "s"(A.p4), "s"(A.p5), "s"(B.p0), "s"(B.p1), "s"(B.p2), "s"(B.p3),
          "s"(B.p4), "s"(B.p5));
    apx = ax; apy = ay; apz = az; bpx = bx; bpy = by; bpz = bz;
}
#endif

__device__ __forceinline__ void pcl_rotate2(f2 x, f2 y, f2 z, const PclPoseRec* __restrict__ pose, f2& opx, f2& opy, f2& opz)
{
    pcl_rotate2(x, y, z, pcl_pose6(pose), opx, opy, opz);
}

template <int FMT, bool DEPTH = false>
__device__ __forceinline__ void pcl_project2_rotated(__amdgpu_buffer_rsrc_t tex, const PclDims& dm, PclProj<FMT>& o,
                                                     __amdgpu_buffer_rsrc_t zb = __amdgpu_buffer_rsrc_t(), int zoff = 0,
                                                     const PclDepthGrid* dg = nullptr);

template <int FMT, bool DEPTH = false>
__device__ __forceinline__ void pcl_project2(f2 x, f2 y, f2 z, const PclPose6& pose,
                                             __amdgpu_buffer_rsrc_t tex, const PclDims& dm, PclProj<FMT>& o,
                                             __amdgpu_buffer_rsrc_t zb = __amdgpu_buffer_rsrc_t(), int zoff = 0, const PclDepthGrid* dg = nullptr)
{
    pcl_rotate2(x, y, z, pose, o.px, o.py, o.pz);
    pcl_project2_rotated<FMT, DEPTH>(tex, dm, o, zb, zoff, dg);
}

__device__ __forceinline__ void pcl_angles2(f2 px, f2 py, f2 pz, f2& rho2, f2& rinv, f2& rs2, f2& phi, f2& half_el)
{
    f2 a = px + F2(1e-6f), b = pz + F2(1e-6f);
    rho2 = pcl_fma2(px, px, py * py);
    f2 rg = rho2 + F2(1e-37f);
    rinv = (f2){__builtin_amdgcn_rsqf(rg.x), __builtin_amdgcn_rsqf(rg.y)};
    f2 rho = rho2 * rinv;
    phi = pcl_atan2_2(py, a);
    f2 s2 = pcl_fma2(b, b, rho2) + F2(1e-37f);
    rs2 = (f2){__builtin_amdgcn_rsqf(s2.x), __builtin_amdgcn_rsqf(s2.y)};
    f2 den = pcl_fma2(s2, rs2, rho);
    half_el = pcl_atan_poly2(b * (f2){__builtin_amdgcn_rcpf(den.x), __builtin_amdgcn_rcpf(den.y)});
}

template <int FMT, bool DEPTH>
__device__ __forceinline__ void pcl_project2_rotated(__amdgpu_buffer_rsrc_t tex, const PclDims& dm, PclProj<FMT>& o, __amdgpu_buffer_rsrc_t zb,
                                                     int zoff, const PclDepthGrid* dg)
{
    f2 phi, half_el;
    pcl_angles2(o.px, o.py, o.pz, o.rho2, o.rinv, o.rs2, phi, half_el);
    if constexpr (DEPTH) {
        int r0, c0, r1, c1;
        pcl_depth_cells2(phi, half_el, *dg, r0, c0, r1, c1);
        o.zq0 = (unsigned)__builtin_amdgcn_raw_buffer_load_b32(zb, (int)(__umul24((unsigned)r0, (unsigned)dg->Wd) + (unsigned)c0) * 4, zoff, 0);
        o.zq1 = (unsigned)__builtin_amdgcn_raw_buffer_load_b32(zb, (int)(__umul24((unsigned)r1, (unsigned)dg->Wd) + (unsigned)c1) * 4, zoff, 0);
    }
    const float lim_phi = 0.99f * 3.14159265358979323846f, lim_hel = 0.2475f * 3.14159265358979323846f;
    f2 phic = {__builtin_amdgcn_fmed3f(phi.x, -lim_phi, lim_phi), __builtin_amdgcn_fmed3f(phi.y, -lim_phi, lim_phi)};
    f2 helc = {__builtin_amdgcn_fmed3f(half_el.x, -lim_hel, lim_hel), __builtin_amdgcn_fmed3f(half_el.y, -lim_hel, lim_hel)};
    f2 ix = pcl_fma2(phic, F2(dm.k_ix), F2(dm.off_x));
    f2 iy = pcl_fma2(helc, F2(2.f * dm.k_iy), F2(dm.off_y));
    pcl_issue_taps(tex, (int)ix.x, (int)iy.x, dm.Wp, o.ta);
    pcl_issue_taps(tex, (int)ix.y, (int)iy.y, dm.Wp, o.tb);
    o.fx = (f2){__builtin_amdgcn_fractf(ix.x), __builtin_amdgcn_fractf(ix.y)};
    o.fy = (f2){__builtin_amdgcn_fractf(iy.x), __builtin_amdgcn_fractf(iy.y)};
    o.in_phi0 = phi.x == phic.x; o.in_phi1 = phi.y == phic.y;
    o.in_th0 = half_el.x == helc.x; o.in_th1 = half_el.y == helc.y;
}

template <bool GRAD, int FMT>
__device__ __forceinline__ void pcl_sample2(const PclProj<FMT>& o, f2 ncr, f2 ncg, f2 ncb, bool valid0, bool valid1,
                                            unsigned long long vmask0, unsigned long long vmask1,
                                            __amdgpu_buffer_rsrc_t tex, const PclDims& dm, f2* acc, int& count)
{
    const f2 px = o.px, py = o.py, pz = o.pz, fx = o.fx, fy = o.fy;
    f2 c[3], dv[3], dtop[3], dbot[3], dhp[3];
    if constexpr (FMT == PCL_PANO_F16) {
        PclBilerp1 ba, bb;
        pcl_bilerp_f16<GRAD>(o.ta, fx.x, fy.x, ba);
        pcl_bilerp_f16<GRAD>(o.tb, fx.y, fy.y, bb);
#pragma unroll
        for (int k = 0; k < 3; k++) {
            f2 top = {ba.top[k], bb.top[k]};
            dv[k] = (f2){ba.bot[k], bb.bot[k]} - top;
            c[k] = pcl_fma2(fy, dv[k], top);
            if (GRAD) dhp[k] = (f2){ba.dh[k], bb.dh[k]};
        }
    } else {
        float ta[12], tb[12];
        pcl_unpack_taps(tex, o.ta, ta);
        pcl_unpack_taps(tex, o.tb, tb);
#pragma unroll
        for (int k = 0; k < 3; k++) {
            f2 t00 = {ta[k], tb[k]}, t01 = {ta[3 + k], tb[3 + k]}, t10 = {ta[6 + k], tb[6 + k]}, t11 = {ta[9 + k], tb[9 + k]};
            dtop[k] = t01 - t00;
            dbot[k] = t11 - t10;
            f2 top = pcl_fma2(fx, dtop[k], t00), bot = pcl_fma2(fx, dbot[k], t10);
            dv[k] = bot - top;
            c[k] = pcl_fma2(fy, dv[k], top);
        }
    }
    float m0 = fmaxf(fmaxf(fabsf(c[0].x), fabsf(c[1].x)), fabsf(c[2].x));
    float m1 = fmaxf(fmaxf(fabsf(c[0].y), fabsf(c[1].y)), fabsf(c[2].y));
    bool keep0 = valid0 && m0 > 0.f, keep1 = valid1 && m1 > 0.f;
    count += __builtin_popcountll(__builtin_amdgcn_fcmpf(m0, 0.f, 2) & vmask0) +
             __builtin_popcountll(__builtin_amdgcn_fcmpf(m1, 0.f, 2) & vmask1);
    f2 d0, d1, d2;
    if (FMT != PCL_PANO_F32) {
        d0 = pcl_fma2(c[0], F2(dm.c_scale), ncr); d1 = pcl_fma2(c[1], F2(dm.c_scale), ncg); d2 = pcl_fma2(c[2], F2(dm.c_scale), ncb);
    } else {
        d0 = c[0] + ncr; d1 = c[1] + ncg; d2 = c[2] + ncb;
    }
    f2 n2 = pcl_fma2(d0, d0, pcl_fma2(d1, d1, d2 * d2));
    f2 ng = n2 + F2(1e-37f);
    f2 rn = {keep0 ? __builtin_amdgcn_rsqf(ng.x) : 0.f, keep1 ? __builtin_amdgcn_rsqf(ng.y) : 0.f};
    acc[0] = pcl_fma2(n2, rn, acc[0]);
    if (GRAD) {
        f2 dh0, dh1, dh2;
        if constexpr (FMT == PCL_PANO_F16) { dh0 = dhp[0]; dh1 = dhp[1]; dh2 = dhp[2]; }
        else {
            dh0 = pcl_fma2(fy, dbot[0] - dtop[0], dtop[0]);
            dh1 = pcl_fma2(fy, dbot[1] - dtop[1], dtop[1]);
            dh2 = pcl_fma2(fy, dbot[2] - dtop[2], dtop[2]);
        }
        f2 sx = pcl_fma2(d0, dh0, pcl_fma2(d1, dh1, d2 * dh2));
        f2 sy = pcl_fma2(d0, dv[0], pcl_fma2(d1, dv[1], d2 * dv[2]));
        f2 rphi = {o.in_phi0 ? rn.x : 0.f, o.in_phi1 ? rn.y : 0.f}, rth = {o.in_th0 ? rn.x : 0.f, o.in_th1 ? rn.y : 0.f};
        f2 dphi = (sx * F2(dm.k_phi)) * rphi, dth = (sy * F2(dm.k_theta)) * rth;
        f2 a = px + F2(1e-6f), b = pz + F2(1e-6f), rho = o.rho2 * o.rinv;
        f2 s1 = pcl_fma2(a, a, py * py);
        f2 ai = dphi * (f2){__builtin_amdgcn_rcpf(s1.x), __builtin_amdgcn_rcpf(s1.y)};
        f2 bi = dth * (o.rs2 * o.rs2);
        f2 k = b * bi * o.rinv;
        f2 g0 = pcl_fma2(k, px, -(py * ai));
        f2 g1 = pcl_fma2(k, py, a * ai);
        f2 g2 = -(rho * bi);
        acc[2] += g0; acc[3] += g1; acc[4] += g2;
        acc[5] = pcl_fma2(py, g2, pcl_fma2(-pz, g1, acc[5]));
        acc[6] = pcl_fma2(pz, g0, pcl_fma2(-px, g2, acc[6]));
        acc[7] = pcl_fma2(px, g1, pcl_fma2(-py, g0, acc[7]));
    }
}
```

Measured before the change: 3567.

## Compute texel byte offsets in float, carry load offsets, pack blue-below texel layout

Tap addresses are now built from float floor and FMA with a precomputed row stride in bytes, which replaces the integer umul24 and fract sequence whenever the padded panorama fits in 2^24 texels. Point-cloud load offsets are carried as byte counters across steps instead of being recomputed each time. For f16 panoramas, the pack kernel stores the blue channel of the row below next to the texel, so the non-fused bilinear path reads blue from the top load alone. Kernel variants multiply through an int-address flag. A glue-reference build is added to compare the two address paths.

```diff
diff --git a/__graft_entry__.py b/__graft_entry__.py
--- a/__graft_entry__.py
+++ b/__graft_entry__.py
@@ -12,6 +12,7 @@
     so = hip_build.build()
     assert os.path.exists(so), so
     assert os.path.exists(hip_build.build_experiments())
+    assert os.path.exists(hip_build.build_glue_reference())
     from oracle import oracle as orc
     orc.build()
     from piccolo_amd import _lib
diff --git a/piccolo_amd/build.py b/piccolo_amd/build.py
--- a/piccolo_amd/build.py
+++ b/piccolo_amd/build.py
@@ -92,5 +92,39 @@
     return build(force=force, verbose=verbose, experiments=True)
 
 
+REF_SO = os.path.join(OUT_DIR, "libpiccolo_hip_ref.so")
+GLUE_SOURCES = ("pcl_loss.hip", "pcl_trim.hip")
+
+
+def build_glue_reference(force=False, verbose=False):
+    exp_so = build_experiments(force=force, verbose=verbose)
+    if not force and os.path.exists(REF_SO) and os.path.getmtime(REF_SO) >= os.path.getmtime(exp_so):
+        return REF_SO
+    obj_dir = os.path.join(OUT_DIR, "obj_ref")
+    os.makedirs(obj_dir, exist_ok=True)
+    base = [hipcc(), "--offload-arch=" + ARCH, "-O3", "-std=c++17", "-fPIC", "-fno-gpu-rdc", "-pthread", "-Wall", "-Wno-unused-function",
+            "-DPCL_EXPERIMENTS", "-DPCL_GLUE_REFERENCE"]
+    objs = []
+    for src in sources():
+        name = os.path.basename(src)
+        if name in GLUE_SOURCES:
+            obj = os.path.join(obj_dir, name[:-4] + ".o")
+            cmd = base + ["-c", src, "-o", obj]
+            if verbose:
+                print(" ".join(cmd), flush=True)
+            subprocess.check_call(cmd)
+        else:
+            obj = os.path.join(OUT_DIR, "obj_exp", name[:-4] + ".o")
+        objs.append(obj)
+    cmd = [hipcc(), "--offload-arch=" + ARCH, "-shared", "-fPIC", "-fno-gpu-rdc", "-pthread", "-o", REF_SO] + objs
+    if verbose:
+        print(" ".join(cmd), flush=True)
+    subprocess.check_call(cmd)
+    return REF_SO
+
+
 if __name__ == "__main__":
-    print(build(force="--force" in sys.argv, verbose=True, experiments="--experiments" in sys.argv))
+    if "--glue-reference" in sys.argv:
+        print(build_glue_reference(force="--force" in sys.argv, verbose=True))
+    else:
+        print(build(force="--force" in sys.argv, verbose=True, experiments="--experiments" in sys.argv))
diff --git a/piccolo_amd/csrc/pcl_device.h b/piccolo_amd/csrc/pcl_device.h
--- a/piccolo_amd/csrc/pcl_device.h
+++ b/piccolo_amd/csrc/pcl_device.h
@@ -59,6 +59,7 @@
     float k_phi, k_theta;
     float c_scale;
     float k_ix, k_iy;
+    float row_b;
 };
 
 __host__ __device__ inline PclDims pcl_make_dims(int H, int W, int pano_format = PCL_PANO_F32)
@@ -72,6 +73,7 @@
     d.c_scale = 1.0f;
     d.k_ix = (float)(-(double)W / (2.0 * 3.14159265358979323846));
     d.k_iy = (float)(-(double)H / 3.14159265358979323846);
+    d.row_b = (pano_format == PCL_PANO_U8 ? 4.0f : pano_format == PCL_PANO_F16 ? 8.0f : 16.0f) * (float)(W + 2);
     if (pano_format == PCL_PANO_U8 || pano_format == PCL_PANO_F16) {
         d.k_phi = (float)(-(double)W / (2.0 * 3.14159265358979323846) / 255.0);
         d.k_theta = (float)((double)H / 3.14159265358979323846 / 255.0);
diff --git a/piccolo_amd/csrc/pcl_loss.hip b/piccolo_amd/csrc/pcl_loss.hip
--- a/piccolo_amd/csrc/pcl_loss.hip
+++ b/piccolo_amd/csrc/pcl_loss.hip
@@ -72,9 +72,13 @@
     return blockIdx.x - (unsigned)pcl_rfl(rm->block0);
 }
 
-template <int G, bool GRAD, int VIS, int FMT, bool FUSED, bool CS = false, bool RM = false>
+template <int G, bool GRAD, int VIS, int FMT, bool FUSED, bool CS = false, bool RM = false, bool FADDR_IN = true>
 __device__ __forceinline__ void pcl_loss_body(const PclLossArgs& a_in, const PclFuseArgs& f_in, const PclRoomTable* rooms = nullptr)
 {
+    constexpr int FADDR = !FADDR_IN || VIS == 1 || (FUSED && FMT == PCL_PANO_F32) ? PCL_ADDR_INT
+                          : (FMT == PCL_PANO_F16 && VIS == 0 && !FUSED) ? PCL_ADDR_FLOAT_ROWV : PCL_ADDR_FLOAT;
+    constexpr bool CARRY = FADDR != PCL_ADDR_INT;
+    constexpr bool BLUE_BELOW = !FUSED;
     PclLossArgs a_rm;
     PclFuseArgs f_rm;
     unsigned bid = blockIdx.x;
@@ -122,18 +126,32 @@
     if (end > (int)a.n) end = (int)a.n;
     const int last = (int)a.n - 1;
 
-    auto load_step = [&](int base, float (&dst)[2][6]) {
-        int j0 = min(base + (int)threadIdx.x, last), j1 = min(base + PCL_BLOCK + (int)threadIdx.x, last);
+    int step_base = begin;
+    int c0 = (int)threadIdx.x * 4 + begin * 4, c1 = c0 + PCL_BLOCK * 4;
+    const int last4 = last * 4, end4 = end * 4;
+    auto load_step = [&](int ahead, float (&dst)[2][6]) {
+        int j0, j1;
+        if constexpr (CARRY) {
+            j0 = min(c0 + ahead * (PCL_STEP * 4), last4); j1 = min(c1 + ahead * (PCL_STEP * 4), last4);
+        } else {
+            j0 = min(step_base + ahead * PCL_STEP + (int)threadIdx.x, last) * 4; j1 = min(step_base + ahead * PCL_STEP + PCL_BLOCK + (int)threadIdx.x, last) * 4;
+        }
 #pragma unroll
         for (int k = 0; k < 6; k++) {
             const int soff = (CS && k >= 3) ? cplane + (k - 3) * plane : k * plane;
-            dst[0][k] = __builtin_bit_cast(float, __builtin_amdgcn_raw_buffer_load_b32(cld, j0 * 4, soff, 0));
-            dst[1][k] = __builtin_bit_cast(float, __builtin_amdgcn_raw_buffer_load_b32(cld, j1 * 4, soff, 0));
+            dst[0][k] = __builtin_bit_cast(float, __builtin_amdgcn_raw_buffer_load_b32(cld, j0, soff, 0));
+            dst[1][k] = __builtin_bit_cast(float, __builtin_amdgcn_raw_buffer_load_b32(cld, j1, soff, 0));
         }
     };
     auto eval_step = [&](int base, const float (&src)[2][6]) {
         const int i0 = base + threadIdx.x, i1 = i0 + PCL_BLOCK;
-        const bool valid0 = i0 < end, valid1 = i1 < end;
+        bool valid0, valid1;
+        if constexpr (CARRY) {
+            valid0 = c0 < end4; valid1 = c1 < end4;
+            c0 += PCL_STEP * 4; c1 += PCL_STEP * 4;
+        } else {
+            valid0 = i0 < end; valid1 = i1 < end;
+        }
         const unsigned long long vmask0 = __builtin_amdgcn_ballot_w64(valid0), vmask1 = __builtin_amdgcn_ballot_w64(valid1);
         f2 x = {src[0][0], src[1][0]}, y = {src[0][1], src[1][1]}, z = {src[0][2], src[1][2]};
         f2 ncr = {src[0][3], src[1][3]}, ncg = {src[0][4], src[1][4]}, ncb = {src[0][5], src[1][5]};
@@ -177,22 +195,22 @@
 #ifndef PCL_NO_ROTATE_PAIR
             if constexpr (G == 2) {
                 pj.px = rot_p[g][0]; pj.py = rot_p[g][1]; pj.pz = rot_p[g][2];
-                pcl_project2_rotated<FMT, VIS == 2>(tg, a.dims, pj, zb, zoff, &a.dgrid);
+                pcl_project2_rotated<FMT, VIS == 2, FADDR>(tg, a.dims, pj, zb, zoff, &a.dgrid);
             } else
 #endif
-            if constexpr (FUSED) pcl_project2<FMT, VIS == 2>(x, y, z, P6[g], tg, a.dims, pj, zb, zoff, &a.dgrid);
-            else pcl_project2<FMT, VIS == 2>(x, y, z, pcl_pose6(pr), tg, a.dims, pj, zb, zoff, &a.dgrid);
+            if constexpr (FUSED) pcl_project2<FMT, VIS == 2, FADDR>(x, y, z, P6[g], tg, a.dims, pj, zb, zoff, &a.dgrid);
+            else pcl_project2<FMT, VIS == 2, FADDR>(x, y, z, pcl_pose6(pr), tg, a.dims, pj, zb, zoff, &a.dgrid);
             if constexpr (VIS == 2) {
                 f2 d2 = pcl_fma2(pj.pz, pj.pz, pj.rho2);
                 const bool v0 = d2.x <= __uint_as_float(pj.zq0), v1 = d2.y <= __uint_as_float(pj.zq1);
                 ok0 = ok0 & v0; ok1 = ok1 & v1;
                 m0 = __builtin_amdgcn_ballot_w64(ok0); m1 = __builtin_amdgcn_ballot_w64(ok1);
             }
-            pcl_sample2<GRAD, FMT>(pj, ncr, ncg, ncb, ok0, ok1, m0, m1, tg, a.dims, acc[g], count[g]);
+            pcl_sample2<GRAD, FMT, BLUE_BELOW>(pj, ncr, ncg, ncb, ok0, ok1, m0, m1, tg, a.dims, acc[g], count[g]);
         }
     };
     float bufA[2][6], bufB[2][6];
-    load_step(begin, bufA);
+    load_step(0, bufA);
     if constexpr (FUSED) {
         static_assert(PCL_BLOCK == PCL_GD_THREADS, "the fused prologue reduces with the epilogue kernel's thread layout");
         __shared__ double gd_rows[(PCL_GD_THREADS / 16) * 2 * G][4];
@@ -214,10 +232,12 @@
     }
 
     for (int base = begin; base < end; base += 2 * PCL_STEP) {
-        load_step(base + PCL_STEP, bufB);
+        step_base = base;
+        load_step(1, bufB);
         eval_step(base, bufA);
         if (base + PCL_STEP < end) {
-            load_step(base + 2 * PCL_STEP, bufA);
+            step_base = base + PCL_STEP;
+            load_step(1, bufA);
             eval_step(base + PCL_STEP, bufB);
         }
     }
@@ -262,40 +282,44 @@
 #endif
 }
 
+#define PCL_INT_ADDR 8
+#define PCL_FMT_OF(F) ((F) & 7)
+#define PCL_FADDR_OF(F) (((F) & PCL_INT_ADDR) == 0)
+
 template <int G, bool GRAD, int VIS, int FMT>
 __global__ void __launch_bounds__(PCL_BLOCK) pcl_loss_kernel(PclLossArgs a)
 {
-    pcl_loss_body<G, GRAD, VIS, FMT, false>(a, PclFuseArgs{});
+    pcl_loss_body<G, GRAD, VIS, PCL_FMT_OF(FMT), false, false, false, PCL_FADDR_OF(FMT)>(a, PclFuseArgs{});
 }
 
 template <int G, int FMT>
 __global__ void __launch_bounds__(PCL_BLOCK) pcl_loss_fused_kernel(PclLossArgs a, PclFuseArgs f)
 {
-    pcl_loss_body<G, true, 0, FMT, true>(a, f);
+    pcl_loss_body<G, true, 0, PCL_FMT_OF(FMT), true, false, false, PCL_FADDR_OF(FMT)>(a, f);
 }
 
 template <int G, int FMT>
 __global__ void __launch_bounds__(PCL_BLOCK) pcl_loss_sets_kernel(PclLossArgs a)
 {
-    pcl_loss_body<G, true, 0, FMT, false, true>(a, PclFuseArgs{});
+    pcl_loss_body<G, true, 0, PCL_FMT_OF(FMT), false, true, false, PCL_FADDR_OF(FMT)>(a, PclFuseArgs{});
 }
 
 template <int G, int FMT>
 __global__ void __launch_bounds__(PCL_BLOCK) pcl_loss_fused_sets_kernel(PclLossArgs a, PclFuseArgs f)
 {
-    pcl_loss_body<G, true, 0, FMT, true, true>(a, f);
+    pcl_loss_body<G, true, 0, PCL_FMT_OF(FMT), true, true, false, PCL_FADDR_OF(FMT)>(a, f);
 }
 
 template <int G, int FMT>
 __global__ void __launch_bounds__(PCL_BLOCK) pcl_loss_rooms_kernel(PclLossArgs a, const PclRoomTable* rooms)
 {
-    pcl_loss_body<G, true, 0, FMT, false, false, true>(a, PclFuseArgs{}, rooms);
+    pcl_loss_body<G, true, 0, PCL_FMT_OF(FMT), false, false, true, PCL_FADDR_OF(FMT)>(a, PclFuseArgs{}, rooms);
 }
 
 template <int G, int FMT>
 __global__ void __launch_bounds__(PCL_BLOCK) pcl_loss_fused_rooms_kernel(PclLossArgs a, PclFuseArgs f, const PclRoomTable* rooms)
 {
-    pcl_loss_body<G, true, 0, FMT, true, false, true>(a, f, rooms);
+    pcl_loss_body<G, true, 0, PCL_FMT_OF(FMT), true, false, true, PCL_FADDR_OF(FMT)>(a, f, rooms);
 }
 
 
@@ -429,6 +453,15 @@
     }
 }
 
+static int pcl_addr_code(int pano_format, int H, int W)
+{
+#ifdef PCL_GLUE_REFERENCE
+    return pano_format | PCL_INT_ADDR;
+#else
+    return (int64_t)(H + 2) * (W + 2) <= PCL_FLOAT_ADDR_MAX_TEXELS ? pano_format : pano_format | PCL_INT_ADDR;
+#endif
+}
+
 int pcl_launch_loss_rooms(const PclRoomTable* rooms, const void* pano, int pano_format, int H, int W, const PclPoseRec* poses, int B, int G,
                           int ngroups, int nblk, float* partials, hipStream_t s, int flip, const PclFuseArgs* fuse)
 {
@@ -439,29 +472,21 @@
     a.poses = poses; a.B = B; a.partials = partials;
     a.ngroups = ngroups; a.flip = flip & 1; a.xcd_groups = 0; a.color_sets = 1;
     const dim3 grid(nblk), blk(PCL_BLOCK);
-    if (fuse) {
-        if (pano_format == PCL_PANO_U8) {
-            if (G == 2) hipLaunchKernelGGL((pcl_loss_fused_rooms_kernel<2, PCL_PANO_U8>), grid, blk, 0, s, a, *fuse, rooms);
-            else hipLaunchKernelGGL((pcl_loss_fused_rooms_kernel<1, PCL_PANO_U8>), grid, blk, 0, s, a, *fuse, rooms);
-        } else if (pano_format == PCL_PANO_F16) {
-            if (G == 2) hipLaunchKernelGGL((pcl_loss_fused_rooms_kernel<2, PCL_PANO_F16>), grid, blk, 0, s, a, *fuse, rooms);
-            else hipLaunchKernelGGL((pcl_loss_fused_rooms_kernel<1, PCL_PANO_F16>), grid, blk, 0, s, a, *fuse, rooms);
-        } else {
-            if (G == 2) hipLaunchKernelGGL((pcl_loss_fused_rooms_kernel<2, PCL_PANO_F32>), grid, blk, 0, s, a, *fuse, rooms);
-            else hipLaunchKernelGGL((pcl_loss_fused_rooms_kernel<1, PCL_PANO_F32>), grid, blk, 0, s, a, *fuse, rooms);
-        }
-    } else {
-        if (pano_format == PCL_PANO_U8) {
-            if (G == 2) hipLaunchKernelGGL((pcl_loss_rooms_kernel<2, PCL_PANO_U8>), grid, blk, 0, s, a, rooms);
-            else hipLaunchKernelGGL((pcl_loss_rooms_kernel<1, PCL_PANO_U8>), grid, blk, 0, s, a, rooms);
-        } else if (pano_format == PCL_PANO_F16) {
-            if (G == 2) hipLaunchKernelGGL((pcl_loss_rooms_kernel<2, PCL_PANO_F16>), grid, blk, 0, s, a, rooms);
-            else hipLaunchKernelGGL((pcl_loss_rooms_kernel<1, PCL_PANO_F16>), grid, blk, 0, s, a, rooms);
-        } else {
-            if (G == 2) hipLaunchKernelGGL((pcl_loss_rooms_kernel<2, PCL_PANO_F32>), grid, blk, 0, s, a, rooms);
-            else hipLaunchKernelGGL((pcl_loss_rooms_kernel<1, PCL_PANO_F32>), grid, blk, 0, s, a, rooms);
-        }
-    }
+#define PCL_ROOMS_CASE(F)                                                                                                    \
+    case F:                                                                                                                  \
+        if (fuse) {                                                                                                          \
+            if (G == 2) hipLaunchKernelGGL((pcl_loss_fused_rooms_kernel<2, F>), grid, blk, 0, s, a, *fuse, rooms);           \
+            else hipLaunchKernelGGL((pcl_loss_fused_rooms_kernel<1, F>), grid, blk, 0, s, a, *fuse, rooms);                  \
+        } else {                                                                                                             \
+            if (G == 2) hipLaunchKernelGGL((pcl_loss_rooms_kernel<2, F>), grid, blk, 0, s, a, rooms);                        \
+            else hipLaunchKernelGGL((pcl_loss_rooms_kernel<1, F>), grid, blk, 0, s, a, rooms);                               \
+        }                                                                                                                    \
+        break;
+    switch (pcl_addr_code(pano_format, H, W)) {
+        PCL_ROOMS_CASE(PCL_PANO_U8) PCL_ROOMS_CASE(PCL_PANO_F16) PCL_ROOMS_CASE(PCL_PANO_F32)
+        PCL_ROOMS_CASE(PCL_PANO_U8 | PCL_INT_ADDR) PCL_ROOMS_CASE(PCL_PANO_F16 | PCL_INT_ADDR) PCL_ROOMS_CASE(PCL_PANO_F32 | PCL_INT_ADDR)
+    }
+#undef PCL_ROOMS_CASE
     PCL_LAUNCH_CHECK();
     return 0;
 }
@@ -498,24 +523,18 @@
     a.xcd_groups = ((flip & 2) != 0 || xg_env == 1) && xg_env != 0 && p.ngroups % 8 == 0 ? 1 : 0;
     int nblk = p.nchunks * p.ngroups;
     const int vis = depth ? 2 : visible != nullptr ? 1 : 0;
-    if (sets) {
-        if (pano_format == PCL_PANO_U8) pcl_launch_sets<PCL_PANO_U8>(a, fuse, p.G, nblk, s);
-        else if (pano_format == PCL_PANO_F16) pcl_launch_sets<PCL_PANO_F16>(a, fuse, p.G, nblk, s);
-        else pcl_launch_sets<PCL_PANO_F32>(a, fuse, p.G, nblk, s);
-        PCL_LAUNCH_CHECK();
-        return 0;
-    }
-    if (fuse) {
-        if (!grad || vis) return PCL_EINVAL;
-        if (pano_format == PCL_PANO_U8) pcl_launch_fused<PCL_PANO_U8>(a, *fuse, p.G, nblk, s);
-        else if (pano_format == PCL_PANO_F16) pcl_launch_fused<PCL_PANO_F16>(a, *fuse, p.G, nblk, s);
-        else pcl_launch_fused<PCL_PANO_F32>(a, *fuse, p.G, nblk, s);
-        PCL_LAUNCH_CHECK();
-        return 0;
-    }
-    if (pano_format == PCL_PANO_U8) pcl_launch_f<PCL_PANO_U8>(a, p.G, nblk, grad, vis, s);
-    else if (pano_format == PCL_PANO_F16) pcl_launch_f<PCL_PANO_F16>(a, p.G, nblk, grad, vis, s);
-    else pcl_launch_f<PCL_PANO_F32>(a, p.G, nblk, grad, vis, s);
+    if (fuse && !sets && (!grad || vis)) return PCL_EINVAL;
+#define PCL_LOSS_CASE(F)                                                \
+    case F:                                                             \
+        if (sets) pcl_launch_sets<F>(a, fuse, p.G, nblk, s);            \
+        else if (fuse) pcl_launch_fused<F>(a, *fuse, p.G, nblk, s);     \
+        else pcl_launch_f<F>(a, p.G, nblk, grad, vis, s);               \
+        break;
+    switch (pcl_addr_code(pano_format, H, W)) {
+        PCL_LOSS_CASE(PCL_PANO_U8) PCL_LOSS_CASE(PCL_PANO_F16) PCL_LOSS_CASE(PCL_PANO_F32)
+        PCL_LOSS_CASE(PCL_PANO_U8 | PCL_INT_ADDR) PCL_LOSS_CASE(PCL_PANO_F16 | PCL_INT_ADDR) PCL_LOSS_CASE(PCL_PANO_F32 | PCL_INT_ADDR)
+    }
+#undef PCL_LOSS_CASE
     PCL_LAUNCH_CHECK();
     return 0;
 }
diff --git a/piccolo_amd/csrc/pcl_pack.hip b/piccolo_amd/csrc/pcl_pack.hip
--- a/piccolo_amd/csrc/pcl_pack.hip
+++ b/piccolo_amd/csrc/pcl_pack.hip
@@ -339,20 +339,24 @@
     int64_t i = (int64_t)blockIdx.x * PCL_BLOCK + threadIdx.x;
     if (i >= (int64_t)Wp * Hp) return;
     int yp = (int)(i / Wp), xp = (int)(i - (int64_t)yp * Wp);
-    float lv[3] = {0.f, 0.f, 0.f};
+    float lv[3] = {0.f, 0.f, 0.f}, below = 0.f;
+    bool bad = false;
     if (yp >= 1 && yp <= H && xp >= 1 && xp <= W) {
         const float* s = img + ((int64_t)(yp - 1) * W + (xp - 1)) * 3;
-        bool bad = false;
 #pragma unroll
         for (int c = 0; c < 3; c++) {
             float f = s[c], k = rintf(f * 255.f);
             bad = bad || !(k >= 0.f && k <= 255.f) || __fdiv_rn(k, 255.f) != f;
             lv[c] = k;
         }
-        if (bad) *not_exact = 1;
-    }
-    h2 rg = {(_Float16)lv[0], (_Float16)lv[1]}, b0 = {(_Float16)lv[2], (_Float16)0.f};
-    pano[i] = (pcl_i2){__builtin_bit_cast(int, rg), __builtin_bit_cast(int, b0)};
+    }
+    if (yp + 1 >= 1 && yp + 1 <= H && xp >= 1 && xp <= W) {
+        float k = rintf(img[((int64_t)yp * W + (xp - 1)) * 3 + 2] * 255.f);
+        below = k >= 0.f && k <= 255.f ? k : 0.f;
+    }
+    if (bad) *not_exact = 1;
+    h2 rg = {(_Float16)lv[0], (_Float16)lv[1]}, bb = {(_Float16)lv[2], (_Float16)below};
+    pano[i] = (pcl_i2){__builtin_bit_cast(int, rg), __builtin_bit_cast(int, bb)};
 }
 
 extern "C" int pcl_pano_pack_f16(const float* img_hwc, int H, int W, void* pano, int* not_exact, void* stream)
diff --git a/piccolo_amd/csrc/pcl_sample_device.h b/piccolo_amd/csrc/pcl_sample_device.h
--- a/piccolo_amd/csrc/pcl_sample_device.h
+++ b/piccolo_amd/csrc/pcl_sample_device.h
@@ -62,22 +62,38 @@
 template <> struct PclTaps<PCL_PANO_F32> { int voff, row; };
 template <> struct PclTaps<PCL_PANO_F16> { pcl_i4 top, bot; };
 
-__device__ __forceinline__ void pcl_issue_taps(__amdgpu_buffer_rsrc_t tex, int x0, int y0, int Wp, PclTaps<PCL_PANO_U8>& o)
-{
-    int voff = (int)(__umul24((unsigned)y0, (unsigned)Wp) + (unsigned)x0) * 4;
+__device__ __forceinline__ void pcl_issue_taps_at(__amdgpu_buffer_rsrc_t tex, int voff, int Wp, PclTaps<PCL_PANO_U8>& o)
+{
     o.top = pcl_texel_pair_u8(tex, voff, 0);
     o.bot = pcl_texel_pair_u8(tex, voff, Wp * 4);
 }
-__device__ __forceinline__ void pcl_issue_taps(__amdgpu_buffer_rsrc_t tex, int x0, int y0, int Wp, PclTaps<PCL_PANO_F16>& o)
-{
-    int voff = (int)(__umul24((unsigned)y0, (unsigned)Wp) + (unsigned)x0) * 8;
+__device__ __forceinline__ void pcl_issue_taps_at(__amdgpu_buffer_rsrc_t tex, int voff, int Wp, PclTaps<PCL_PANO_F16>& o)
+{
     o.top = __builtin_amdgcn_raw_buffer_load_b128(tex, voff, 0, 0);
     o.bot = __builtin_amdgcn_raw_buffer_load_b128(tex, voff, Wp * 8, 0);
 }
-__device__ __forceinline__ void pcl_issue_taps(__amdgpu_buffer_rsrc_t tex, int x0, int y0, int Wp, PclTaps<PCL_PANO_F32>& o)
-{
-    o.voff = (int)(__umul24((unsigned)y0, (unsigned)Wp) + (unsigned)x0) * 16;
+__device__ __forceinline__ void pcl_issue_taps_at(__amdgpu_buffer_rsrc_t, int voff, int Wp, PclTaps<PCL_PANO_F32>& o)
+{
+    o.voff = voff;
     o.row = Wp * 16;
+}
+template <int FMT>
+__device__ __forceinline__ void pcl_issue_taps(__amdgpu_buffer_rsrc_t tex, int x0, int y0, int Wp, PclTaps<FMT>& o)
+{
+    pcl_issue_taps_at(tex, (int)(__umul24((unsigned)y0, (unsigned)Wp) + (unsigned)x0) * pcl_texel_bytes(FMT), Wp, o);
+}
+#define PCL_FLOAT_ADDR_MAX_TEXELS ((int64_t)1 << 24)
+#define PCL_ADDR_INT 0
+#define PCL_ADDR_FLOAT 1
+#define PCL_ADDR_FLOAT_ROWV 2
+template <int FMT, int FADDR>
+__device__ __forceinline__ void pcl_tap_offsets2(f2 ix, f2 iy, const PclDims& dm, f2& fx, f2& fy, int& voff0, int& voff1)
+{
+    const float row_b = FADDR == PCL_ADDR_FLOAT_ROWV ? (float)(dm.Wp * pcl_texel_bytes(FMT)) : dm.row_b;
+    f2 flx = {__builtin_floorf(ix.x), __builtin_floorf(ix.y)}, fly = {__builtin_floorf(iy.x), __builtin_floorf(iy.y)};
+    f2 off = pcl_fma2(flx, F2((float)pcl_texel_bytes(FMT)), fly * F2(row_b));
+    voff0 = (int)(unsigned)off.x; voff1 = (int)(unsigned)off.y;
+    fx = ix - flx; fy = iy - fly;
 }
 __device__ __forceinline__ void pcl_unpack_taps(__amdgpu_buffer_rsrc_t, const PclTaps<PCL_PANO_U8>& r, float t[12])
 {
@@ -108,24 +124,42 @@
     return r;
 }
 struct PclBilerp1 { float top[3], bot[3], dh[3]; };
-template <bool GRAD>
+template <bool GRAD, bool BLUE_BELOW>
 __device__ __forceinline__ void pcl_bilerp_f16(const PclTaps<PCL_PANO_F16>& r, float fx, float fy, PclBilerp1& o)
 {
     typedef _Float16 pcl_h8 __attribute__((ext_vector_type(8)));
     pcl_h8 tv = __builtin_bit_cast(pcl_h8, r.top), bv = __builtin_bit_cast(pcl_h8, r.bot);
     pcl_h2 t00a = __builtin_shufflevector(tv, tv, 0, 1), t00b = __builtin_shufflevector(tv, tv, 2, 3);
     pcl_h2 t01a = __builtin_shufflevector(tv, tv, 4, 5), t01b = __builtin_shufflevector(tv, tv, 6, 7);
-    pcl_h2 t10a = __builtin_shufflevector(bv, bv, 0, 1), t10b = __builtin_shufflevector(bv, bv, 2, 3);
-    pcl_h2 t11a = __builtin_shufflevector(bv, bv, 4, 5), t11b = __builtin_shufflevector(bv, bv, 6, 7);
-    pcl_h2 dta = t01a - t00a, dtb = t01b - t00b, dba = t11a - t10a, dbb = t11b - t10b;
-    o.top[0] = pcl_mix_lo(fx, dta, t00a); o.bot[0] = pcl_mix_lo(fx, dba, t10a);
-    o.top[1] = pcl_mix_hi(fx, dta, t00a); o.bot[1] = pcl_mix_hi(fx, dba, t10a);
-    o.top[2] = pcl_mix_lo(fx, dtb, t00b); o.bot[2] = pcl_mix_lo(fx, dbb, t10b);
-    if (GRAD) {
-        pcl_h2 dda = dba - dta, ddb = dbb - dtb;
-        o.dh[0] = pcl_mix_lo(fy, dda, dta);
-        o.dh[1] = pcl_mix_hi(fy, dda, dta);
-        o.dh[2] = pcl_mix_lo(fy, ddb, dtb);
+    pcl_h2 t10a = __builtin_shufflevector(bv, bv, 0, 1), t11a = __builtin_shufflevector(bv, bv, 4, 5);
+#ifdef PCL_GLUE_REFERENCE
+    constexpr bool BELOW = false;
+#else
+    constexpr bool BELOW = BLUE_BELOW;
+#endif
+    if constexpr (!BELOW) {
+        pcl_h2 t10b = __builtin_shufflevector(bv, bv, 2, 3), t11b = __builtin_shufflevector(bv, bv, 6, 7);
+        pcl_h2 dta = t01a - t00a, dtb = t01b - t00b, dba = t11a - t10a, dbb = t11b - t10b;
+        o.top[0] = pcl_mix_lo(fx, dta, t00a); o.bot[0] = pcl_mix_lo(fx, dba, t10a);
+        o.top[1] = pcl_mix_hi(fx, dta, t00a); o.bot[1] = pcl_mix_hi(fx, dba, t10a);
+        o.top[2] = pcl_mix_lo(fx, dtb, t00b); o.bot[2] = pcl_mix_lo(fx, dbb, t10b);
+        if (GRAD) {
+            pcl_h2 dda = dba - dta, ddb = dbb - dtb;
+            o.dh[0] = pcl_mix_lo(fy, dda, dta);
+            o.dh[1] = pcl_mix_hi(fy, dda, dta);
+            o.dh[2] = pcl_mix_lo(fy, ddb, dtb);
+        }
+    } else {
+        pcl_h2 dta = t01a - t00a, dtb = t01b - t00b, dba = t11a - t10a;
+        o.top[0] = pcl_mix_lo(fx, dta, t00a); o.bot[0] = pcl_mix_lo(fx, dba, t10a);
+        o.top[1] = pcl_mix_hi(fx, dta, t00a); o.bot[1] = pcl_mix_hi(fx, dba, t10a);
+        o.top[2] = pcl_mix_lo(fx, dtb, t00b); o.bot[2] = pcl_mix_hi(fx, dtb, t00b);
+        if (GRAD) {
+            pcl_h2 dda = dba - dta, ddb = __builtin_shufflevector(dtb, dtb, 1, 0) - dtb;
+            o.dh[0] = pcl_mix_lo(fy, dda, dta);
+            o.dh[1] = pcl_mix_hi(fy, dda, dta);
+            o.dh[2] = pcl_mix_lo(fy, ddb, dtb);
+        }
     }
 }
 
@@ -217,18 +251,18 @@
     pcl_rotate2(x, y, z, pcl_pose6(pose), opx, opy, opz);
 }
 
-template <int FMT, bool DEPTH = false>
+template <int FMT, bool DEPTH = false, int FADDR = PCL_ADDR_INT>
 __device__ __forceinline__ void pcl_project2_rotated(__amdgpu_buffer_rsrc_t tex, const PclDims& dm, PclProj<FMT>& o,
                                                      __amdgpu_buffer_rsrc_t zb = __amdgpu_buffer_rsrc_t(), int zoff = 0,
                                                      const PclDepthGrid* dg = nullptr);
 
-template <int FMT, bool DEPTH = false>
+template <int FMT, bool DEPTH = false, int FADDR = PCL_ADDR_INT>
 __device__ __forceinline__ void pcl_project2(f2 x, f2 y, f2 z, const PclPose6& pose,
                                              __amdgpu_buffer_rsrc_t tex, const PclDims& dm, PclProj<FMT>& o,
                                              __amdgpu_buffer_rsrc_t zb = __amdgpu_buffer_rsrc_t(), int zoff = 0, const PclDepthGrid* dg = nullptr)
 {
     pcl_rotate2(x, y, z, pose, o.px, o.py, o.pz);
-    pcl_project2_rotated<FMT, DEPTH>(tex, dm, o, zb, zoff, dg);
+    pcl_project2_rotated<FMT, DEPTH, FADDR>(tex, dm, o, zb, zoff, dg);
 }
 
 __device__ __forceinline__ void pcl_angles2(f2 px, f2 py, f2 pz, f2& rho2, f2& rinv, f2& rs2, f2& phi, f2& half_el)
@@ -245,7 +279,7 @@
     half_el = pcl_atan_poly2(b * (f2){__builtin_amdgcn_rcpf(den.x), __builtin_amdgcn_rcpf(den.y)});
 }
 
-template <int FMT, bool DEPTH>
+template <int FMT, bool DEPTH, int FADDR>
 __device__ __forceinline__ void pcl_project2_rotated(__amdgpu_buffer_rsrc_t tex, const PclDims& dm, PclProj<FMT>& o, __amdgpu_buffer_rsrc_t zb,
                                                      int zoff, const PclDepthGrid* dg)
 {
@@ -262,15 +296,22 @@
     f2 helc = {__builtin_amdgcn_fmed3f(half_el.x, -lim_hel, lim_hel), __builtin_amdgcn_fmed3f(half_el.y, -lim_hel, lim_hel)};
     f2 ix = pcl_fma2(phic, F2(dm.k_ix), F2(dm.off_x));
     f2 iy = pcl_fma2(helc, F2(2.f * dm.k_iy), F2(dm.off_y));
-    pcl_issue_taps(tex, (int)ix.x, (int)iy.x, dm.Wp, o.ta);
-    pcl_issue_taps(tex, (int)ix.y, (int)iy.y, dm.Wp, o.tb);
-    o.fx = (f2){__builtin_amdgcn_fractf(ix.x), __builtin_amdgcn_fractf(ix.y)};
-    o.fy = (f2){__builtin_amdgcn_fractf(iy.x), __builtin_amdgcn_fractf(iy.y)};
+    if constexpr (FADDR != PCL_ADDR_INT) {
+        int voff0, voff1;
+        pcl_tap_offsets2<FMT, FADDR>(ix, iy, dm, o.fx, o.fy, voff0, voff1);
+        pcl_issue_taps_at(tex, voff0, dm.Wp, o.ta);
+        pcl_issue_taps_at(tex, voff1, dm.Wp, o.tb);
+    } else {
+        pcl_issue_taps(tex, (int)ix.x, (int)iy.x, dm.Wp, o.ta);
+        pcl_issue_taps(tex, (int)ix.y, (int)iy.y, dm.Wp, o.tb);
+        o.fx = (f2){__builtin_amdgcn_fractf(ix.x), __builtin_amdgcn_fractf(ix.y)};
+        o.fy = (f2){__builtin_amdgcn_fractf(iy.x), __builtin_amdgcn_fractf(iy.y)};
+    }
     o.in_phi0 = phi.x == phic.x; o.in_phi1 = phi.y == phic.y;
     o.in_th0 = half_el.x == helc.x; o.in_th1 = half_el.y == helc.y;
 }
 
-template <bool GRAD, int FMT>
+template <bool GRAD, int FMT, bool BLUE_BELOW = true>
 __device__ __forceinline__ void pcl_sample2(const PclProj<FMT>& o, f2 ncr, f2 ncg, f2 ncb, bool valid0, bool valid1,
                                             unsigned long long vmask0, unsigned long long vmask1,
                                             __amdgpu_buffer_rsrc_t tex, const PclDims& dm, f2* acc, int& count)
@@ -279,8 +320,8 @@
     f2 c[3], dv[3], dtop[3], dbot[3], dhp[3];
     if constexpr (FMT == PCL_PANO_F16) {
         PclBilerp1 ba, bb;
-        pcl_bilerp_f16<GRAD>(o.ta, fx.x, fy.x, ba);
-        pcl_bilerp_f16<GRAD>(o.tb, fx.y, fy.y, bb);
+        pcl_bilerp_f16<GRAD, BLUE_BELOW>(o.ta, fx.x, fy.x, ba);
+        pcl_bilerp_f16<GRAD, BLUE_BELOW>(o.tb, fx.y, fy.y, bb);
 #pragma unroll
         for (int k = 0; k < 3; k++) {
             f2 top = {ba.top[k], bb.top[k]};
```

Result: no change. 3585, median of 6 (+0.5%).
